# flkraus/bayesian-yolov3

Measured on AMD Instinct MI355X. Metric: img/s at T=30 MC-dropout, 608x608, higher is better.
Workload: dtype f32 via split-f16 (hi+lo fp16 pairs, 3 fp16 MFMA products, fp32 accumulate)

## Files before the change

### bayesian-yolov3_amd/byolo/_lib.py

```python
import ctypes
import os

_HERE = os.path.dirname(os.path.abspath(__file__))
LIB_PATH = os.environ.get("BYOLO_LIB") or os.path.join(_HERE, "libbyolo.so")

OK, ERR_ARG, ERR_STATE, ERR_HIP, ERR_NOMEM, ERR_RANGE = 0, -1, -2, -3, -4, -5
DET_STANDARD, DET_ALEATORIC, DET_EPISTEMIC = 0, 1, 2
NMS_AGNOSTIC, NMS_TWO_CLASS, NMS_PER_CLASS = 0, 1, 2
NMS_MAX_CLASSES = 128
NORM_BN, NORM_DROPOUT = 1, 2
AUG_SATURATION, AUG_BRIGHTNESS, AUG_HUE = 1, 2, 3
AUG_COLORED_SALT_N_PEPPER, AUG_SALT_N_PEPPER, AUG_GAUSSIAN = 1, 2, 3


class ByoloError(RuntimeError):
    def __init__(self, code, msg):
        super().__init__("libbyolo error %d: %s" % (code, msg))
        self.code = code


class Cfg(ctypes.Structure):
    _fields_ = [("img_h", ctypes.c_int32), ("img_w", ctypes.c_int32), ("img_c", ctypes.c_int32),
                ("cls_cnt", ctypes.c_int32), ("drop_prob", ctypes.c_float), ("max_out", ctypes.c_int32),
                ("iou_thresh", ctypes.c_float), ("nms_mode", ctypes.c_int32), ("keep_all_outputs", ctypes.c_int32)]


class PlanOpts(ctypes.Structure):
    _fields_ = [(n, ctypes.c_int32) for n in (
        "struct_bytes", "graphs", "serialize_convs", "serialize_heads", "dedup", "lowmain", "kx3", "p1", "b2b", "kx3_wide", "wino_split", "wino_split_min_c",
        "wino_split_bn", "wino_split_rounds", "winograd", "wino_fused", "stream1x1", "gemm_stream", "ksplit", "streamk",
        "plain_epilogue", "wshift_per_layer", "nms_general", "wino_split_persist", "wino_split_feed")] + [(n, ctypes.c_float) for n in (
        "wino_split_min_gflop", "wino_split_chunk_mb", "wino_min_gflop", "wino_chunk_mb", "wino_min_ratio")]


class AugPlan(ctypes.Structure):
    _fields_ = [(n, ctypes.c_int32) for n in ("y0", "x0", "ch", "cw", "row0", "rescale", "flip", "blur_k", "color_op", "noise_op")] + \
               [("color_param", ctypes.c_float), ("noise_param", ctypes.c_float), ("noise_key", ctypes.c_uint64)]


EVAL_MAX_GT, EVAL_MAX_UNC, EVAL_RECORD_HEAD = 1024, 16, 7


class EvalCfg(ctypes.Structure):
    _fields_ = [(n, ctypes.c_int32) for n in ("struct_bytes", "row_len", "obj_idx", "cls_start_idx", "cls_cnt", "n_unc")] + \
               [("unc_cols", ctypes.c_int32 * EVAL_MAX_UNC), ("iou_thresh", ctypes.c_float), ("min_score", ctypes.c_float)]


EVAL_LOC_WORDS, EVAL_LOC_MAX_LAYERS, EVAL_LOC_MAX_PRIORS = 6, 8, 16


class EvalLocCfg(ctypes.Structure):
    _fields_ = [(n, ctypes.c_int32) for n in ("struct_bytes", "layer_col", "prior_col", "n_layers")] + \
               [(n, ctypes.c_int32 * EVAL_LOC_MAX_LAYERS) for n in ("lh", "lw", "n_priors")] + \
               [(n, (ctypes.c_float * EVAL_LOC_MAX_PRIORS) * EVAL_LOC_MAX_LAYERS) for n in ("prior_w", "prior_h")]


EVAL_LADDER_MAX = 16


class EvalLadderCfg(ctypes.Structure):
    _fields_ = [("struct_bytes", ctypes.c_int32), ("n_thr", ctypes.c_int32), ("thresholds", ctypes.c_float * EVAL_LADDER_MAX)]


EVAL_SUBSETS_MAX = 16


class EvalSubsetsCfg(ctypes.Structure):
    _fields_ = [("struct_bytes", ctypes.c_int32), ("n_subsets", ctypes.c_int32), ("lo", ctypes.c_float * EVAL_SUBSETS_MAX),
                ("hi", ctypes.c_float * EVAL_SUBSETS_MAX), ("img_h", ctypes.c_float), ("ignore_thresh", ctypes.c_float),
                ("height_slack", ctypes.c_float), ("ignore_other_classes", ctypes.c_int32)]


class EvalSummary(ctypes.Structure):
    _fields_ = [(n, ctypes.c_int32) for n in ("struct_bytes", "overflow", "record_words", "reserved")] + \
               [(n, ctypes.c_int64) for n in ("n_records", "n_seen", "n_images")]


VOTE_NONE, VOTE_ALE, VOTE_EPI, VOTE_TOTAL = 0, 1, 2, 3


class VoteCfg(ctypes.Structure):
    _fields_ = [("struct_bytes", ctypes.c_int32), ("var", ctypes.c_int32)] + \
               [(n, ctypes.c_float) for n in ("sigma_t", "iou_min", "min_score", "var_floor")] + \
               [("ale_col", ctypes.c_int32), ("epi_col", ctypes.c_int32)]


SOFT_NMS_LINEAR, SOFT_NMS_GAUSSIAN = 0, 1
SOFT_NMS_RESIDENT = 8192


class SoftNmsCfg(ctypes.Structure):
    _fields_ = [("struct_bytes", ctypes.c_int32), ("method", ctypes.c_int32)] + \
               [(n, ctypes.c_float) for n in ("sigma", "iou_soft", "iou_hard", "min_score")]


VAR_RECAL_ALE, VAR_RECAL_EPI, VAR_RECAL_TOTAL = 1, 2, 3
VAR_RECAL_SCALE, VAR_RECAL_POWER = 0, 1
VAR_RECAL_FITTED, VAR_RECAL_SCALE_FALLBACK, VAR_RECAL_IDENTITY, VAR_RECAL_EMPTY = 0, 1, 2, 3
VAR_RECAL_TABLE_BYTES, VAR_RECAL_FIT_WORDS = 8192, 10


class VarRecalCfg(ctypes.Structure):
    _fields_ = [(n, ctypes.c_int32) for n in ("struct_bytes", "kind", "target", "n_layers")] + \
               [("n_priors", ctypes.c_int32 * EVAL_LOC_MAX_LAYERS)] + \
               [(n, ((ctypes.c_double * 4) * EVAL_LOC_MAX_PRIORS) * EVAL_LOC_MAX_LAYERS) for n in ("a", "b")]


SCORE_RECAL_MAX_K, SCORE_RECAL_MAX_GROUPS, SCORE_RECAL_TABLE_BYTES, SCORE_RECAL_FIT_WORDS = 8, 80, 5120, 36
SCORE_RECAL_BY_ALL, SCORE_RECAL_BY_CLASS = 0, 1
SCORE_RECAL_F_BIAS, SCORE_RECAL_F_LOGIT, SCORE_RECAL_F_LOG_HEIGHT, SCORE_RECAL_F_COL_ID, SCORE_RECAL_F_COL_LOG = 0, 1, 2, 3, 4
SCORE_RECAL_FIT, SCORE_RECAL_IDENTITY, SCORE_RECAL_EMPTY = 0, 1, 2


class ScoreRecalCfg(ctypes.Structure):
    _fields_ = [(n, ctypes.c_int32) for n in ("struct_bytes", "kind", "cls_cnt", "by", "K")] + \
               [(n, ctypes.c_int32 * SCORE_RECAL_MAX_K) for n in ("feat_kind", "feat_col")] + [("reserved", ctypes.c_int32)] + \
               [("w", (ctypes.c_double * SCORE_RECAL_MAX_K) * SCORE_RECAL_MAX_GROUPS)]


_i32, _i64, _f32 = ctypes.c_int32, ctypes.c_int64, ctypes.c_float
_vp, _cp, _sz, _u64 = ctypes.c_void_p, ctypes.c_char_p, ctypes.c_size_t, ctypes.c_uint64
_P = ctypes.POINTER

PROTOTYPES = {
    "byolo_create": (_i32, [_P(Cfg), _i32, _P(_vp)]),
    "byolo_destroy": (_i32, [_vp]),
    "byolo_last_error": (_cp, [_vp]),
    "byolo_version": (_cp, []),
    "byolo_add_conv": (_i32, [_vp, _cp, _i32, _i32, _i32, _i32]),
    "byolo_add_residual": (_i32, [_vp, _i32]),
    "byolo_add_route": (_i32, [_vp, _P(_i32), _i32]),
    "byolo_add_upsample": (_i32, [_vp]),
    "byolo_add_stack": (_i32, [_vp, _i32]),
    "byolo_add_detection": (_i32, [_vp, _cp, _i32, _P(_f32)]),
    "byolo_mark_backbone_end": (_i32, [_vp]),
    "byolo_num_params": (_i32, [_vp]),
    "byolo_param_info": (_i32, [_vp, _i32, _P(_cp), _P(_i32), _P(_i64)]),
    "byolo_set_param": (_i32, [_vp, _cp, _vp, _i64]),
    "byolo_get_param": (_i32, [_vp, _cp, _vp, _i64]),
    "byolo_finalize": (_i32, [_vp]),
    "byolo_num_layers": (_i32, [_vp]),
    "byolo_num_boxes": (_i32, [_vp, _P(_i64), _P(_i32)]),
    "byolo_workspace_bytes": (_i32, [_vp, _i32, _i32, _P(_sz)]),
    "byolo_forward": (_i32, [_vp, _vp, _i32, _i32, _u64, _i32, _vp, _vp, _sz, _vp, _vp, _vp, _vp, _vp]),
    "byolo_num_dropout": (_i32, [_vp]),
    "byolo_mask_layout": (_i32, [_vp, _i32, _i32, _i32, _P(_i64), _P(_i64)]),
    "byolo_set_async": (_i32, [_vp, _i32]),
    "byolo_status": (_i32, [_vp, _vp, _P(ctypes.c_uint32), _P(_i32)]),
    "byolo_clear_status": (_i32, [_vp, _vp]),
    "byolo_precision_note": (_cp, [_vp]),
    "byolo_set_first_image": (_i32, [_vp, _i64]),
    "byolo_max_images": (_i32, [_vp, _i32, _P(_i32)]),
    "byolo_layer_output": (_i32, [_vp, _i32, _P(_vp), _P(_i64)]),
    "byolo_copy_layer_output": (_i32, [_vp, _i32, _vp, _i64, _vp]),
    "byolo_set_precision": (_i32, [_vp, _i32]),
    "byolo_get_precision": (_i32, [_vp]),
    "byolo_decode": (_i32, [_vp, _i32, _vp, _i32, _i32, _i32, _i32, _P(_f32), _i32, _vp, _i64, _i64, _vp]),
    "byolo_epistemic_stats": (_i32, [_vp, _vp, _i32, _i32, _i32, _i32, _vp, _vp, _vp, _vp, _vp]),
    "byolo_nms_workspace_bytes": (_sz, [_i32, _i64]),
    "byolo_nms_workspace_bytes_ex": (_sz, [_i32, _i64, _i32, _i32]),
    "byolo_nms_class_counts": (_i32, [_vp, _vp, _i32, _i32, _vp]),
    "byolo_sort_nms": (_i32, [_vp, _vp, _i32, _i64, _i32, _i32, _i32, _i32, _i32, _f32, _vp, _sz, _vp, _vp, _vp, _vp]),
    "byolo_calibrate_bn": (_i32, [_vp, _vp, _i32, _vp, _sz, _vp]),
    "byolo_set_profiling": (_i32, [_vp, _i32]),
    "byolo_resume_profiling": (_i32, [_vp, _i32]),
    "byolo_stage_ms": (_i32, [_vp, _P(_f32)]),
    "byolo_set_profile_depth": (_i32, [_vp, _i32]),
    "byolo_select_profile": (_i32, [_vp, _i32]),
    "byolo_num_steps": (_i32, [_vp]),
    "byolo_step_profile": (_i32, [_vp, _i32, _P(_i32), _P(_i32), _P(_i64), _P(_f32), _P(ctypes.c_double)]),
    "byolo_step_split": (_i32, [_vp, _i32, _P(_i32), _P(_i32)]),
    "byolo_flops": (_i32, [_vp, _i32, _i32, _P(ctypes.c_double)]),
    "byolo_crc32c": (ctypes.c_uint32, [_vp, _sz]),
    "byolo_abi_version": (_i32, []),
    "byolo_get_plan_opts": (_i32, [_vp, _P(PlanOpts)]),
    "byolo_set_plan_opts": (_i32, [_vp, _P(PlanOpts)]),
    "byolo_graph_stats": (_i32, [_vp, _P(_i32), _P(_i64), _P(_i64), _P(_i64)]),
    "byolo_plan_num": (_i32, [_vp, _i32, _i32, _i32, _P(_i32), _P(_i32), _P(_i64)]),
    "byolo_plan_step": (_i32, [_vp, _i32, _P(_i32), _P(_i32), _P(_i32), _P(_i32)]),
    "byolo_plan_tensor": (_i32, [_vp, _i32, _P(_i64), _P(_i64), _P(_i32)]),
    "byolo_set_tshard": (_i32, [_vp, _i32, _i32]),
    "byolo_finish_tshard": (_i32, [_vp, _vp, _i32, _i32, _vp]),
    "byolo_normalize_u8": (_i32, [_vp, _vp, _i64, _vp, _vp]),
    "byolo_copy_status": (_i32, [_vp, _vp, _vp]),
# ... 92 lines not shown
```

### bayesian-yolov3_amd/csrc/byolo_api.hip

```cpp
#include "byolo_internal.h"
#include <cfloat>

static thread_local std::string g_err;

int32_t byolo_fail(byolo_t* h, int32_t code, const char* fmt, ...) {
    char buf[1024];
    va_list ap; va_start(ap, fmt); vsnprintf(buf, sizeof buf, fmt, ap); va_end(ap);
    if (h) h->err = buf; else g_err = buf;
    return code;
}

extern "C" const char* byolo_version(void) { return "byolo 0.7 (gfx950; fp32 MFMA and split-f16 MFMA; abi 7)"; }
extern "C" int32_t byolo_abi_version(void) { return BYOLO_ABI_VERSION; }

extern "C" const char* byolo_last_error(const byolo_t* h) { return h ? h->err.c_str() : g_err.c_str(); }

static void plan_opts_defaults(byolo_plan_opts& o);
static void plan_opts_from_env(byolo_plan_opts& o);

extern "C" int32_t byolo_create(const byolo_cfg* cfg, int32_t device, byolo_t** out) {
    if (!cfg || !out) return fail(nullptr, BYOLO_ERR_ARG, "byolo_create: null argument");
    if (cfg->img_h <= 0 || cfg->img_w <= 0 || cfg->img_c <= 0)
        return fail(nullptr, BYOLO_ERR_ARG, "byolo_create: invalid image size");
    if (cfg->img_h % 32 || cfg->img_w % 32)
        return fail(nullptr, BYOLO_ERR_ARG, "byolo_create: full_img_size must be a multiple of 32 (yolov3.py:207-208)");
    if (cfg->cls_cnt < 1 || cfg->cls_cnt > byk::BYOLO_MAX_CLASSES)
        return fail(nullptr, BYOLO_ERR_ARG, "byolo_create: cls_cnt outside 1 .. 128");
    if (cfg->max_out < 1 || cfg->max_out > 2048) return fail(nullptr, BYOLO_ERR_ARG, "byolo_create: max_out out of [1,2048]");
    if (!(cfg->drop_prob >= 0.f && cfg->drop_prob < 1.f)) return fail(nullptr, BYOLO_ERR_ARG, "byolo_create: drop_prob");
    byolo_t* h = new (std::nothrow) byolo();
    if (!h) return fail(nullptr, BYOLO_ERR_NOMEM, "byolo_create: out of host memory");
    h->cfg = *cfg;
    h->device = device;
    plan_opts_defaults(h->opts);
    plan_opts_from_env(h->opts);
    h->dedup = h->opts.dedup != 0;
    if (const char* e = getenv("BYOLO_PRECISION")) h->precision = (!strcmp(e, "f32") || !strcmp(e, "0")) ? 0 : 1;
    h->prec_requested = h->precision;
    *out = h;
    return BYOLO_OK;
}

static void plan_opts_defaults(byolo_plan_opts& o) {
    memset(&o, 0, sizeof o);
    o.struct_bytes = (int32_t)sizeof o;
    o.graphs = 1; o.serialize_convs = 1; o.serialize_heads = 1; o.dedup = 1; o.lowmain = 1; o.kx3 = 1; o.p1 = 1; o.b2b = 1; o.kx3_wide = 0;
    o.wino_split = 1; o.wino_split_min_c = 256; o.wino_split_bn = 0; o.wino_split_rounds = 0;
    o.winograd = 1; o.wino_fused = 1; o.stream1x1 = 1; o.gemm_stream = 1; o.ksplit = -1; o.streamk = 1; o.plain_epilogue = 1; o.wino_split_persist = 0; o.wino_split_feed = 3;
    o.wino_split_min_gflop = 30.f; o.wino_split_chunk_mb = 1500.f; o.wino_min_gflop = 10.f; o.wino_chunk_mb = 800.f; o.wino_min_ratio = 80.f;
}
static void plan_opts_from_env(byolo_plan_opts& o) {
    auto geti = [](const char* name, int32_t& v) { if (const char* e = getenv(name)) v = atoi(e); };
    auto getf = [](const char* name, float& v) { if (const char* e = getenv(name)) v = (float)atof(e); };
    geti("BYOLO_GRAPHS", o.graphs); geti("BYOLO_SERIALIZE_CONVS", o.serialize_convs); geti("BYOLO_SERIALIZE_HEADS", o.serialize_heads);
    if (const char* e = getenv("BYOLO_NO_DEDUP")) o.dedup = atoi(e) ? 0 : 1;
    geti("BYOLO_LOWMAIN", o.lowmain); geti("BYOLO_KX3", o.kx3); geti("BYOLO_P1", o.p1); geti("BYOLO_B2B", o.b2b); geti("BYOLO_KX3_WIDE", o.kx3_wide);
    geti("BYOLO_WINO_SPLIT", o.wino_split); geti("BYOLO_WINO_SPLIT_MIN_C", o.wino_split_min_c); geti("BYOLO_WINO_SPLIT_BN", o.wino_split_bn);
    geti("BYOLO_WINO_SPLIT_ROUNDS", o.wino_split_rounds); geti("BYOLO_WINOGRAD", o.winograd);
    geti("BYOLO_WINO_FUSED", o.wino_fused); geti("BYOLO_STREAM1X1", o.stream1x1); geti("BYOLO_GEMM_STREAM", o.gemm_stream);
    geti("BYOLO_KSPLIT", o.ksplit); geti("BYOLO_STREAMK", o.streamk); geti("BYOLO_PLAIN_EPILOGUE", o.plain_epilogue); geti("BYOLO_WINO_SPLIT_PERSIST", o.wino_split_persist); geti("BYOLO_WINO_SPLIT_FEED", o.wino_split_feed);
    geti("BYOLO_WSHIFT_PER_LAYER", o.wshift_per_layer); geti("BYOLO_NMS_GENERAL", o.nms_general);
    getf("BYOLO_WINO_SPLIT_MIN_GFLOP", o.wino_split_min_gflop); getf("BYOLO_WINO_SPLIT_CHUNK_MB", o.wino_split_chunk_mb);
    getf("BYOLO_WINO_MIN_GFLOP", o.wino_min_gflop); getf("BYOLO_WINO_CHUNK_MB", o.wino_chunk_mb); getf("BYOLO_WINO_MIN_RATIO", o.wino_min_ratio);
}

static void drop_graphs(byolo_t* h) {
    bool any = false;
    for (auto& g : h->graphs) any = any || g.exec;
    if (any) (void)hipDeviceSynchronize();
    for (auto& g : h->graphs) if (g.exec) (void)hipGraphExecDestroy(g.exec);
    h->graphs.clear();
}

extern "C" int32_t byolo_get_plan_opts(const byolo_t* h, byolo_plan_opts* out) {
    if (!h || !out) return fail(const_cast<byolo_t*>(h), BYOLO_ERR_ARG, "byolo_get_plan_opts: null argument");
    *out = h->opts;
    out->struct_bytes = (int32_t)sizeof *out;
    return BYOLO_OK;
}

extern "C" int32_t byolo_set_plan_opts(byolo_t* h, const byolo_plan_opts* o) {
    if (!h || !o) return fail(h, BYOLO_ERR_ARG, "byolo_set_plan_opts: null argument");
    if (o->struct_bytes != (int32_t)sizeof *o) return fail(h, BYOLO_ERR_ARG, "byolo_set_plan_opts: struct_bytes %d, this library's byolo_plan_opts has %d (include/byolo.h)", o->struct_bytes, (int)sizeof *o);
    if (o->graphs < 0 || o->graphs > 2 || o->serialize_convs < 0 || o->serialize_convs > 2 || o->b2b < 0 || o->b2b > 2 || o->kx3_wide < 0 || o->kx3_wide > 2 ||
        o->wino_split < 0 || o->wino_split > 2 || o->winograd < 0 || o->winograd > 2 || o->wino_fused < 0 || o->wino_fused > 2 || o->stream1x1 < 0 || o->stream1x1 > 2 ||
        o->streamk < 0 || o->streamk > 2 || o->ksplit < -1 || o->ksplit > 64 || (o->wino_split_bn != 0 && o->wino_split_bn != 128 && o->wino_split_bn != 256) ||
        o->wino_split_rounds < 0 || o->wino_split_persist < 0 || o->wino_split_persist > 2 || o->wino_split_feed < 0 || o->wino_split_feed > 3 || !(o->wino_split_chunk_mb > 0.f) || !(o->wino_chunk_mb > 0.f) || !(o->wino_split_min_gflop >= 0.f) || !(o->wino_min_gflop >= 0.f) || !(o->wino_min_ratio >= 0.f))
        return fail(h, BYOLO_ERR_ARG, "byolo_set_plan_opts: a field outside its range (include/byolo.h)");
    const byolo_plan_opts& c = h->opts;
    const bool repack = (o->wshift_per_layer != 0) != (c.wshift_per_layer != 0) || (o->dedup != 0) != (c.dedup != 0) || (o->lowmain != 0) != (c.lowmain != 0) || (o->kx3 != 0) != (c.kx3 != 0) || (o->p1 != 0) != (c.p1 != 0);
    h->opts = *o;
    h->dedup = o->dedup != 0;
    invalidate_plan(h);
    if (h->d_blob || !h->graphs.empty()) { HIPCHK(h, hipSetDevice(h->device)); drop_graphs(h); }
    if (repack && h->lowered) { h->lowered = false; h->finalized = false; }
    return BYOLO_OK;
}

extern "C" int32_t byolo_graph_stats(const byolo_t* h, int32_t* n_graphs, int64_t* replays, int64_t* captures, int64_t* updates) {
    if (!h) return BYOLO_ERR_ARG;
    int n = 0; for (const auto& g : h->graphs) n += g.exec != nullptr;
    if (n_graphs) *n_graphs = n;
    if (replays) *replays = h->graph_replays;
    if (captures) *captures = h->graph_captures;
    if (updates) *updates = h->graph_updates;
    return BYOLO_OK;
}

extern "C" int32_t byolo_set_precision(byolo_t* h, int32_t precision) {
    if (!h) return fail(nullptr, BYOLO_ERR_ARG, "byolo_set_precision: null handle");
    if (precision != BYOLO_PREC_F32 && precision != BYOLO_PREC_SPLIT_F16) return fail(h, BYOLO_ERR_ARG, "byolo_set_precision: unknown precision %d", precision);
    h->prec_requested = precision;
    if (precision == BYOLO_PREC_F32) h->prec_note.clear();
    if (precision != h->precision) { h->precision = precision; h->prec_note.clear(); h->finalized = false; h->plan.B = -1; h->plan.T = -1; ++h->plan_epoch; }
    return BYOLO_OK;
}
extern "C" int32_t byolo_get_precision(const byolo_t* h) { return h ? h->precision : BYOLO_ERR_ARG; }

extern "C" int32_t byolo_destroy(byolo_t* h) {
    if (!h) return BYOLO_OK;
    bool on_device = h->d_blob || h->d_ones || h->d_status || !h->graphs.empty() || h->cap_stream;
    for (auto& ps : h->prof) on_device = on_device || ps.ev[0] || !ps.step_ev.empty();
    if (on_device) {
        (void)hipSetDevice(h->device);
        drop_graphs(h);
        if (h->cap_stream) (void)hipStreamDestroy(h->cap_stream);
        if (h->d_blob) (void)hipFree(h->d_blob);
        if (h->d_ones) (void)hipFree(h->d_ones);
        if (h->d_zeros) (void)hipFree(h->d_zeros);
        if (h->ev_convs) (void)hipEventDestroy(h->ev_convs);
        if (h->d_status) (void)hipFree(h->d_status);
        if (h->pc_own) (void)hipFree(h->pc_own);
        if (h->vn_own) (void)hipFree(h->vn_own);
        if (h->vr.dev) (void)hipFree(h->vr.dev);
        if (h->sr.dev) (void)hipFree(h->sr.dev);
        if (h->sr_own) (void)hipFree(h->sr_own);
        if (h->h_status) (void)hipHostFree(h->h_status);
        for (auto& ps : h->prof) {
            for (auto& e : ps.ev) if (e) (void)hipEventDestroy(e);
            for (auto& e : ps.step_ev) (void)hipEventDestroy(e);
        }
    }
    delete h;
    return BYOLO_OK;
}

static int add_param(byolo_t* h, const std::string& name, std::vector<int64_t> shape, float fill) {
    if (h->pindex.count(name)) return -1;
    Param p; p.name = name; p.shape = std::move(shape);
    p.data.assign((size_t)p.count(), fill);
    h->params.push_back(std::move(p));
    h->pindex[name] = (int)h->params.size() - 1;
    return (int)h->params.size() - 1;
}

static int resolve_ref(const byolo_t* h, int r) {
    const int n = (int)h->layers.size();
    const int a = r < 0 ? n + r : r;
    return (a < 0 || a >= n) ? -2 : a;
}

static void input_shape(const byolo_t* h, int prev, int& C, int& H, int& W, bool& stacked) {
    if (prev < 0) { C = h->cfg.img_c; H = h->cfg.img_h; W = h->cfg.img_w; stacked = false; }
    else { const Layer& l = h->layers[prev]; C = l.C; H = l.H; W = l.W; stacked = l.stacked; }
}

static int32_t begin_add(byolo_t* h, const char* what) {
    if (!h) return fail(nullptr, BYOLO_ERR_ARG, "%s: null handle", what);
    if (h->lowered) return fail(h, BYOLO_ERR_STATE, "%s: graph is frozen after byolo_finalize", what);
    return BYOLO_OK;
}

static constexpr int MAX_CHANNELS = 1 << 16;
static constexpr int64_t MAX_KERNEL_WEIGHTS = (int64_t)1 << 28;

static int32_t add_conv_impl(byolo_t* h, const char* scope, int32_t filters, int32_t ksize, int32_t stride, int32_t norm_flags) {
    int32_t rc = begin_add(h, "byolo_add_conv"); if (rc) return rc;
    if (!scope || !(ksize == 1 || ksize == 3)) return fail(h, BYOLO_ERR_ARG, "byolo_add_conv: invalid kernel size");
    if (!(stride == 1 || stride == 2)) return fail(h, BYOLO_ERR_ARG, "byolo_add_conv: invalid strides");
    if (stride == 2 && ksize != 3) return fail(h, BYOLO_ERR_ARG, "byolo_add_conv: invalid kernel size (layers.py:629)");
    if (filters < 1) return fail(h, BYOLO_ERR_ARG, "byolo_add_conv: filters < 1");
    if (filters > MAX_CHANNELS) return fail(h, BYOLO_ERR_ARG, "byolo_add_conv: more than %d filters", MAX_CHANNELS);
    if (!(norm_flags & BYOLO_NORM_BN)) return fail(h, BYOLO_ERR_ARG, "byolo_add_conv: BN-less conv layers are not on this path");
    Layer l; l.op = OP_CONV; l.scope = scope; l.filters = filters; l.ksize = ksize; l.stride = stride; l.norm = norm_flags;
    l.prev = (int)h->layers.size() - 1;
    int C, H, W; bool st; input_shape(h, l.prev, C, H, W, st);
    if (stride == 2 && ((H | W) & 1)) return fail(h, BYOLO_ERR_ARG, "byolo_add_conv: stride 2 needs even input size");
    if ((int64_t)ksize * ksize * C * filters > MAX_KERNEL_WEIGHTS)
        return fail(h, BYOLO_ERR_ARG, "byolo_add_conv: a kernel of %lld weights (limit 2^28)", (long long)ksize * ksize * C * filters);
    l.Cin = C; l.C = filters; l.H = H / stride; l.W = W / stride; l.stacked = st;
    const std::string s(scope);
    l.p_kernel = add_param(h, s + "/conv2d/kernel", {ksize, ksize, C, filters}, 0.f);
    l.p_gamma = add_param(h, s + "/batch_normalization/gamma", {filters}, 1.f);
    l.p_beta = add_param(h, s + "/batch_normalization/beta", {filters}, 0.f);
    l.p_mean = add_param(h, s + "/batch_normalization/moving_mean", {filters}, 0.f);
    l.p_var = add_param(h, s + "/batch_normalization/moving_variance", {filters}, 1.f);
    if (l.p_kernel < 0 || l.p_gamma < 0) return fail(h, BYOLO_ERR_ARG, "byolo_add_conv: duplicate scope '%s'", scope);
    if (norm_flags & BYOLO_NORM_DROPOUT) l.drop_ordinal = h->n_dropout++;
    h->layers.push_back(l);
    return (int32_t)h->layers.size() - 1;
}
extern "C" int32_t byolo_add_conv(byolo_t* h, const char* scope, int32_t filters, int32_t ksize, int32_t stride,
                                  int32_t norm_flags) {
    return guarded(h, "byolo_add_conv", [&] { return add_conv_impl(h, scope, filters, ksize, stride, norm_flags); });
}

extern "C" int32_t byolo_add_residual(byolo_t* h, int32_t shortcut) {
    int32_t rc = begin_add(h, "byolo_add_residual"); if (rc) return rc;
    Layer l; l.op = OP_RESIDUAL; l.prev = (int)h->layers.size() - 1;
    const int a = resolve_ref(h, shortcut);
    if (a < 0 || l.prev < 0) return fail(h, BYOLO_ERR_ARG, "byolo_add_residual: bad shortcut %d", shortcut);
    const Layer& x = h->layers[l.prev]; const Layer& s = h->layers[a];
    if (x.C != s.C || x.H != s.H || x.W != s.W || x.stacked != s.stacked)
        return fail(h, BYOLO_ERR_ARG, "byolo_add_residual: shape mismatch");
    l.ref[0] = a; l.nref = 1; l.C = x.C; l.H = x.H; l.W = x.W; l.stacked = x.stacked;
    h->layers.push_back(l);
    return (int32_t)h->layers.size() - 1;
}

extern "C" int32_t byolo_add_route(byolo_t* h, const int32_t* routes, int32_t n) {
    int32_t rc = begin_add(h, "byolo_add_route"); if (rc) return rc;
    if (!routes || n >= 3) return fail(h, BYOLO_ERR_ARG, "byolo_add_route: too many routes");
    if (n < 1) return fail(h, BYOLO_ERR_ARG, "byolo_add_route: too few routes");
    Layer l; l.op = OP_ROUTE; l.prev = (int)h->layers.size() - 1; l.nref = n;
    for (int i = 0; i < n; ++i) {
        l.ref[i] = resolve_ref(h, routes[i]);
        if (l.ref[i] < 0) return fail(h, BYOLO_ERR_ARG, "byolo_add_route: bad route %d", routes[i]);
    }
    const Layer& a = h->layers[l.ref[0]];
    l.C = a.C; l.H = a.H; l.W = a.W; l.stacked = a.stacked;
    if (n == 2) {
        const Layer& b = h->layers[l.ref[1]];
        if (a.H != b.H || a.W != b.W || a.stacked != b.stacked)
            return fail(h, BYOLO_ERR_ARG, "byolo_add_route: concat shape mismatch");
        l.C = a.C + b.C;
        if (l.C > MAX_CHANNELS) return fail(h, BYOLO_ERR_ARG, "byolo_add_route: more than %d channels", MAX_CHANNELS);
    }
    h->layers.push_back(l);
    return (int32_t)h->layers.size() - 1;
}
// ... 319 lines not shown
    p.N = layer_pitch(l); p.Npad = st.Npad; p.ldc = layer_pitch(l);
    p.cin_tiles = (st.c_hi - st.c_lo) / 32; p.KT = l.ksize * l.ksize * p.cin_tiles;
    p.wpk = dptr(h, st.w_off);
    p.epi = raw_epi(h, st.layer);
    p.dst = h->plan.off[st.out_tensor] >= 0 ? reinterpret_cast<float*>(ws + h->plan.off[st.out_tensor]) : nullptr;
    p.src0_bytes = (uint32_t)((uint64_t)nsrc[0] * Hs[0] * Wsz[0] * Cs[0] * 4);
    p.src1_bytes = Cs[1] ? (uint32_t)((uint64_t)nsrc[1] * Hs[1] * Wsz[1] * Cs[1] * 4) : p.src0_bytes;
    p.w_bytes = (uint32_t)((uint64_t)p.KT * p.Npad * 32 * 4);
    p.d_hw = make_fastdiv((uint32_t)(p.Hout * p.Wout)); p.d_wout = make_fastdiv((uint32_t)p.Wout);
    p.d_sdiv0 = make_fastdiv((uint32_t)sdiv[0]); p.d_sdiv1 = make_fastdiv((uint32_t)sdiv[1]);
    p.rep = st.mode == STEP_REP ? T : 1;
    p.split = h->precision != 1 ? 0 : (!l.direct ? 1 : ((l.prev >= 0 ? 1 : 0) | (l.op == OP_DETECTION ? 0 : 2)));
    if (p.split && st.kx3) { p.kx3 = 1; p.KT = 3 * p.cin_tiles; }
    else if (p.split && st.p1) p.kx3 = 2;
    if (st.mode == STEP_MAIN) {
        p.addend = reinterpret_cast<const float*>(ws + h->plan.off[st.addend_tensor]);
        p.addend_T = l.stacked ? T : 1;
    } else { p.addend = nullptr; p.addend_T = 1; }
    p.d_addT = make_fastdiv((uint32_t)p.addend_T);
    p.no_plain = h->opts.plain_epilogue == 0;
}

static void fill_finish(const byolo_t* h, const Step& st, char* ws, int B, int T, int mode, FinishParams& f) {
    const Layer& l = h->layers[st.layer];
    memset(&f, 0, sizeof f);
    f.low = reinterpret_cast<const float*>(ws + h->plan.off[st.low_tensor]);
    f.part = st.addend_tensor >= 0 ? reinterpret_cast<const float*>(ws + h->plan.off[st.addend_tensor]) : nullptr;
    f.dst = h->plan.off[st.out_tensor] >= 0 ? reinterpret_cast<float*>(ws + h->plan.off[st.out_tensor]) : nullptr;
    f.T = l.stacked ? T : 1; f.S = B * f.T; f.H = l.H; f.W = l.W; f.N = l.filters;
    f.mode = mode;
    f.epi = raw_epi(h, st.layer); f.epi.flags = 0;
    f.d_hw = make_fastdiv((uint32_t)(l.H * l.W / 4)); f.d_w = make_fastdiv((uint32_t)(l.W / 2));
    f.d_n4 = make_fastdiv((uint32_t)(l.filters / 4)); f.d_T = make_fastdiv((uint32_t)f.T);
}

static int32_t run_aux_step(byolo_t* h, const Step& s, const ConvParams& p, hipStream_t st) {
    const Layer& l = h->layers[s.layer];
    if (s.mode == STEP_GATHER) { HIPCHK(h, launch_view_gather(p, st)); }
    else { HIPCHK(h, launch_tensor_add(p.src0, p.src1, p.dst, (int64_t)p.M * l.C, h->precision == 1, st, p.epi.status, s.layer)); }
    return BYOLO_OK;
}

static int32_t next_event(byolo_t* h, hipStream_t st, int* idx) {
    byolo::ProfSlot& ps = h->wslot();
    while ((int)ps.step_ev.size() <= ps.n_ev) { hipEvent_t e; HIPCHK(h, hipEventCreate(&e)); ps.step_ev.push_back(e); }
    HIPCHK(h, hipEventRecord(ps.step_ev[ps.n_ev], st));
    *idx = ps.n_ev++;
    return BYOLO_OK;
}

static int32_t mark_launch(byolo_t* h, int layer, int variant, int64_t m, int64_t n, int64_t k, double algo, hipStream_t st,
                           int ksplit = 1, int split_tiles = 0) {
    byolo::ProfSlot& ps = h->wslot();
    int e; int32_t rc = next_event(h, st, &e); if (rc) return rc;
    if (ps.last_main >= 0) ps.launches[ps.last_main].ev_end = e;
    ps.last_main = (int)ps.launches.size();
    ps.launches.push_back({layer, variant, m, n, k, algo, ksplit, split_tiles, e, -1});
    return BYOLO_OK;
}

static int32_t run_winograd(byolo_t* h, const Step& s, const Layer& l, const ConvParams& c, const WinoPlan& wp, int tile,
                            double algo_flops, char* ws, hipStream_t st) {
    const bool prof = h->profiling >= 2;
    int32_t rc;
    const int S = c.M / (l.H * l.W), tt = wp.th * wp.tw;
    float* V = reinterpret_cast<float*>(ws + h->plan.wino_off);
    float* Mb = reinterpret_cast<float*>(ws + h->plan.wino_off + wp.v_bytes);
    for (int s0 = 0; s0 < S; s0 += wp.chunk) {
        const int ns = std::min(wp.chunk, S - s0);
        WinoParams w; memset(&w, 0, sizeof w);
        w.x = c.src0; w.v = V; w.m = Mb; w.y = c.dst;
        w.residual = (c.epi.flags & EPI_RESIDUAL) ? c.residual : nullptr;
        w.epi = c.epi;
        w.H = l.H; w.W = l.W; w.C = c.C0; w.N = c.N; w.th = wp.th; w.tw = wp.tw;
        w.s0 = s0; w.P = ns * tt; w.P_pad = (int)align_up((size_t)w.P, 128);
        w.d_tt = make_fastdiv((uint32_t)tt); w.d_tw = make_fastdiv((uint32_t)wp.tw);
        w.d_c4 = make_fastdiv((uint32_t)(c.C0 / 4)); w.d_n4 = make_fastdiv((uint32_t)(c.N / 4));
        if (prof && (rc = mark_launch(h, s.layer, -2, w.P, c.C0, 0, 0.0, st))) return rc;
        HIPCHK(h, launch_wino_input(w, st));

        const int rows = 16 * w.P_pad;
        if (wp.fused) {
            WinoFusedParams f; memset(&f, 0, sizeof f);
            f.v = V; f.v_bytes = (uint32_t)((uint64_t)rows * c.C0 * 4);
            f.w = dptr(h, s.wino_off); f.wstride = (uint32_t)((size_t)(c.C0 / 32) * c.N * 32 * 4); f.w_bytes = 16u * f.wstride;
            f.y = c.dst; f.residual = w.residual; f.epi = c.epi;
            f.C = c.C0; f.N = c.N; f.KT = c.C0 / 32; f.n_tiles = c.N / 64;
            f.H = l.H; f.W = l.W; f.th = wp.th; f.tw = wp.tw; f.s0 = s0; f.P = w.P;
            const int RT = w.P_pad / 128;
            f.slots = 512 / f.n_tiles; f.q = RT / f.slots; f.rem = RT % f.slots;
            f.xi_stride = (uint32_t)((uint64_t)w.P_pad * c.C0 * 4);
            f.d_ntiles = make_fastdiv((uint32_t)f.n_tiles); f.d_tt = w.d_tt; f.d_tw = w.d_tw;
            if (prof && (rc = mark_launch(h, s.layer, 130, rows, c.N, c.C0, algo_flops * ns / S, st))) return rc;
            HIPCHK(h, launch_wino_fused(f, st));
            continue;
        }
        if (h->opts.gemm_stream != 0 && gemm_stream_ok(c.C0, c.N)) {
            GemmStreamParams q; memset(&q, 0, sizeof q);
            q.a = V; q.a_bytes = (uint32_t)((uint64_t)rows * c.C0 * 4);
            q.w = dptr(h, s.wino_off); q.wstride = (uint32_t)((size_t)(c.C0 / 32) * c.N * 32 * 4); q.w_bytes = 16u * q.wstride;
            q.dst = Mb; q.C = c.C0; q.N = c.N; q.KT = c.C0 / 32; q.n_tiles = c.N / 128;
            q.RT = w.P_pad / 128;
            const int R = 16 * q.RT;
            q.slots = 512 / q.n_tiles; q.q = R / q.slots; q.rem = R % q.slots;
            q.d_ntiles = make_fastdiv((uint32_t)q.n_tiles); q.d_RT = make_fastdiv((uint32_t)q.RT);
            q.kind = 0; q.epi = raw_epi(h, s.layer); q.M = rows; q.Npad = c.N; q.ldc = c.N;
            if (prof && (rc = mark_launch(h, s.layer, 129, rows, c.N, c.C0, algo_flops * ns / S, st))) return rc;
            HIPCHK(h, launch_gemm_stream(q, st));
            if (prof && (rc = mark_launch(h, s.layer, -3, w.P, c.N, 0, 0.0, st))) return rc;
            HIPCHK(h, launch_wino_output(w, st));
            continue;
        }
        ConvParams g; memset(&g, 0, sizeof g);
        g.src0 = V; g.src1 = V; g.C0 = c.C0; g.C1 = 0;
        g.src0_bytes = g.src1_bytes = (uint32_t)((uint64_t)rows * c.C0 * 4);
        g.Hs0 = g.Hs1 = 1; g.Ws0 = g.Ws1 = rows; g.sdiv0 = g.sdiv1 = 1;
        g.Hin = 1; g.Win = rows; g.Hout = 1; g.Wout = rows; g.ksize = 1; g.stride = 1; g.pad = 0;
        g.M = rows; g.N = c.N; g.Npad = c.Npad; g.ldc = c.N; g.cin_tiles = c.C0 / 32; g.KT = g.cin_tiles;
        g.wpk = dptr(h, s.wino_off);
        g.wino_rows = (uint32_t)w.P_pad; g.d_wino = make_fastdiv((uint32_t)w.P_pad);
        g.wino_wstride = (uint32_t)((size_t)g.cin_tiles * c.Npad * 32 * 4);
        g.w_bytes = 16u * g.wino_wstride;
        g.epi = raw_epi(h, s.layer); g.rep = 1; g.addend_T = 1;
        g.dst = Mb;
        g.d_hw = make_fastdiv((uint32_t)rows); g.d_wout = make_fastdiv((uint32_t)rows);
        g.d_sdiv0 = g.d_sdiv1 = g.d_addT = make_fastdiv(1u);
        const ConvSplit sp = conv_plan_split(rows, c.Npad, g.KT, tile, 1.0, h->opts.ksplit, h->opts.streamk);
        if (conv_split_slab_bytes(sp, tile) <= h->plan.slab_bytes) {
            g.full_tiles = sp.full_tiles; g.split_tiles = sp.split_tiles; g.split_blocks = sp.split_blocks; g.ksplit = sp.ksplit;
            g.sk_grid = sp.sk_grid;
            g.slabs = c.slabs; g.slab_bytes = (uint32_t)conv_split_slab_bytes(sp, tile); g.counters = c.counters;
        }
        if (prof && (rc = mark_launch(h, s.layer, conv_tile_bn(tile), rows, c.N, c.C0, algo_flops * ns / S, st, g.sk_grid > 0 ? -g.sk_grid : (g.ksplit > 1 ? g.ksplit : 1), g.split_tiles))) return rc;
        HIPCHK(h, launch_conv_igemm(g, tile, st));
        if (prof && (rc = mark_launch(h, s.layer, -3, w.P, c.N, 0, 0.0, st))) return rc;
        HIPCHK(h, launch_wino_output(w, st));
    }
    return BYOLO_OK;
}

static int32_t run_wino_split(byolo_t* h, const Step& s, const Layer& l, const ConvParams& c, const WinoPlan& wp, double algo_flops,
                              char* ws, hipStream_t st, const WinoParams* feed = nullptr) {
    const bool prof = h->profiling >= 2;
    int32_t rc;
    const int S = c.M / (l.H * l.W), tt = wp.th * wp.tw;
    float* V = reinterpret_cast<float*>(ws + h->plan.wino_off);
    const bool drop = c.epi.flags & EPI_DROPOUT;
    for (int s0 = 0; s0 < S; s0 += wp.chunk) {
        const int ns = std::min(wp.chunk, S - s0);
        WinoParams w; memset(&w, 0, sizeof w);
        if (feed) w = *feed;
        w.x = feed ? nullptr : c.src0; w.v = V;
        w.H = l.H; w.W = l.W; w.C = c.C0; w.N = c.N; w.th = wp.th; w.tw = wp.tw;
        w.s0 = s0; w.P = ns * tt; w.P_pad = (int)align_up((size_t)w.P, 128);
        w.d_tt = make_fastdiv((uint32_t)tt); w.d_tw = make_fastdiv((uint32_t)wp.tw);
        w.d_c4 = make_fastdiv((uint32_t)(c.C0 / 4)); w.d_n4 = make_fastdiv((uint32_t)(c.N / 4));
        w.vmul = 1.f / ACT_SCALE;
        if (prof && (rc = mark_launch(h, s.layer, -4, w.P, c.C0, 0, 0.0, st))) return rc;
        HIPCHK(h, launch_wino_split_input(w, st));
        WinoSplitParams f; memset(&f, 0, sizeof f);
        const uint64_t rows = (uint64_t)16 * w.P_pad;
        f.v = V; f.v_bytes = (uint32_t)(rows * c.C0 * 4); f.xi_stride = (uint32_t)((uint64_t)w.P_pad * c.C0 * 4);
        f.w = dptr(h, s.wino_off); f.w_bytes = (uint32_t)((size_t)16 * c.C0 * c.N * 4);
        f.y = c.dst; f.residual = (c.epi.flags & EPI_RESIDUAL) ? c.residual : nullptr;
        f.epi = c.epi; f.epi.scale = dptr(h, drop ? l.wscalek_off : l.wscale_off);
        f.C = c.C0; f.N = c.N; f.KT = c.C0 / 32; f.n_tiles = c.N / wp.bn; f.bn = wp.bn;
        f.H = l.H; f.W = l.W; f.th = wp.th; f.tw = wp.tw; f.s0 = s0; f.P = w.P; f.P_pad = w.P_pad;
        f.bm = wp.bm; f.units = (w.P_pad / wp.bm) * f.n_tiles;
        const int chunk_idx = s0 / wp.chunk;
        f.persist = (h->opts.wino_split_persist == 2 && c.counters && chunk_idx < CNT_PER_STEP / 8) ? 2 : (h->opts.wino_split_persist ? 1 : 0);
        f.claims = c.counters ? c.counters + 8 * chunk_idx : nullptr;
        f.d_ntiles = make_fastdiv((uint32_t)f.n_tiles); f.d_tt = w.d_tt; f.d_tw = w.d_tw;
        if (prof && (rc = mark_launch(h, s.layer, 140, (int64_t)rows, c.N, c.C0, algo_flops * ns / S, st, 1, wp.bn))) return rc;
        HIPCHK(h, launch_wino_split(f, st));
    }
    return BYOLO_OK;
}

static int32_t run_decode(byolo_t* h, char* ws, float* boxes, int B, int T, hipStream_t st, int mode = 0) {
    for (const auto& l : h->layers) {
        if (l.op != OP_DETECTION) continue;
        DecodeParams d; memset(&d, 0, sizeof d);
        d.mode = mode;
        if (mode && l.det_kind != BYOLO_DET_EPISTEMIC) return fail(h, BYOLO_ERR_ARG, "T sharding (byolo_set_tshard) is defined for epistemic detection layers");
        d.raw = mode == 2 ? nullptr : reinterpret_cast<const float*>(ws + h->plan.off[l.out_tensor]);
        d.boxes = boxes; d.lh = l.H; d.lw = l.W; d.C = h->cfg.cls_cnt;
        d.n_total = h->n_boxes; d.box_base = l.box_base; d.layer_id = l.det_id; d.ld = layer_pitch(l);
        d.status = h->precision == 1 ? h->d_status : nullptr;
        for (int k = 0; k < 3; ++k) { d.ph[k] = l.priors[2 * k]; d.pw[k] = l.priors[2 * k + 1]; }
        if (l.det_kind == BYOLO_DET_EPISTEMIC) { d.B = B; d.T = l.stacked ? T : 1; }
        else { d.B = l.stacked ? B * T : B; d.T = 1; }
        if (l.det_kind != BYOLO_DET_EPISTEMIC && l.stacked && T > 1)
            return fail(h, BYOLO_ERR_ARG, "byolo_forward: non-epistemic decode of a stacked (T>1) detection layer");
        HIPCHK(h, launch_decode(l.det_kind, d, st));
    }
    return BYOLO_OK;
}

static int64_t mask_layout(const byolo_t* h, int B, int T, int ordinal, int64_t* elements) {
    int64_t off = 0;
    for (const auto& l : h->layers) {
        if (l.drop_ordinal < 0) continue;
        const int64_t n = (l.stacked ? (int64_t)B * T : B) * l.H * l.W * l.filters;
        if (l.drop_ordinal == ordinal) { if (elements) *elements = n; return off; }
        off += (n + 31) / 32 * 32;
    }
    if (elements) *elements = 0;
    return off;
}

extern "C" int32_t byolo_num_dropout(const byolo_t* h) { return h ? h->n_dropout : BYOLO_ERR_ARG; }

static int32_t mask_layout_impl(byolo_t* h, int32_t B, int32_t T, int32_t ordinal, int64_t* bit_offset, int64_t* elements) {
    if (!h) return fail(nullptr, BYOLO_ERR_ARG, "byolo_mask_layout: null handle");
    if (!h->lowered) { int32_t rc = lower(h); if (rc) return rc; }
    if (B < 1 || T < 1 || ordinal < 0 || ordinal > h->n_dropout) return fail(h, BYOLO_ERR_ARG, "byolo_mask_layout: bad argument");
    int64_t n = 0;
    const int64_t off = mask_layout(h, B, T, ordinal, &n);
    if (bit_offset) *bit_offset = off;
    if (elements) *elements = n;
    return BYOLO_OK;
}
extern "C" int32_t byolo_mask_layout(byolo_t* h, int32_t B, int32_t T, int32_t ordinal, int64_t* bit_offset, int64_t* elements) {
    return guarded(h, "byolo_mask_layout", [&] { return mask_layout_impl(h, B, T, ordinal, bit_offset, elements); });
}

static int32_t read_status(byolo_t* h, hipStream_t st, unsigned* flags, unsigned* layer) {
    if (!h->d_status) { *flags = 0; *layer = 0xFFFFFFFFu; return BYOLO_OK; }
    HIPCHK(h, hipMemcpyAsync(h->h_status, h->d_status, 2 * sizeof(unsigned), hipMemcpyDeviceToHost, st));
    HIPCHK(h, hipStreamSynchronize(st));
    *flags = h->h_status[0]; *layer = h->h_status[1];
    return BYOLO_OK;
}
static int32_t range_error(byolo_t* h, const char* what, unsigned flags, unsigned layer) {
    const char* scope = layer < h->layers.size() ? h->layers[layer].scope.c_str() : "?";
    if (flags & 1u)
        return fail(h, BYOLO_ERR_RANGE, "%s: an output of layer %u ('%s') exceeds the split-f16 range (|activation| > %.0f); the reference's float32 "
                    "tensor (lib_yolo/layers.py:550) holds it -- run this model with byolo_set_precision(BYOLO_PREC_F32)", what, layer, scope, 65504.0 / ACT_SCALE);
    return fail(h, BYOLO_ERR_RANGE, "%s: a raw detection output is inf / NaN (non-finite activations upstream, or weights the float32 reference overflows on as well)", what);
}

extern "C" int32_t byolo_set_async(byolo_t* h, int32_t on) {
    if (!h) return fail(nullptr, BYOLO_ERR_ARG, "byolo_set_async: null handle");
    h->async_status = on != 0;
    return BYOLO_OK;
}

extern "C" int32_t byolo_status(byolo_t* h, void* stream, uint32_t* flags, int32_t* layer) {
    if (!h) return fail(nullptr, BYOLO_ERR_ARG, "byolo_status: null handle");
    if (!h->finalized) return fail(h, BYOLO_ERR_STATE, "byolo_status: call byolo_finalize first");
    HIPCHK(h, hipSetDevice(h->device));
    unsigned f = 0, l = 0xFFFFFFFFu;
    int32_t rc = read_status(h, reinterpret_cast<hipStream_t>(stream), &f, &l); if (rc) return rc;
    if (flags) *flags = f;
    if (layer) *layer = (f & 1u) ? (int32_t)l : -1;
    return f ? range_error(h, "byolo_status", f, l) : BYOLO_OK;
}

extern "C" int32_t byolo_clear_status(byolo_t* h, void* stream) {
    if (!h) return fail(nullptr, BYOLO_ERR_ARG, "byolo_clear_status: null handle");
    if (!h->d_status) return BYOLO_OK;
    HIPCHK(h, hipSetDevice(h->device));
    hipStream_t st = reinterpret_cast<hipStream_t>(stream);
    HIPCHK(h, hipMemsetAsync(h->d_status, 0, sizeof(unsigned), st));
    HIPCHK(h, hipMemsetAsync(h->d_status + 1, 0xFF, sizeof(unsigned), st));
    return BYOLO_OK;
}

extern "C" int32_t byolo_copy_status(byolo_t* h, uint32_t* d_out, void* stream) {
    if (!h || !d_out) return fail(h, BYOLO_ERR_ARG, "byolo_copy_status: null argument");
    if (!h->finalized) return fail(h, BYOLO_ERR_STATE, "byolo_copy_status: call byolo_finalize first");
    HIPCHK(h, hipSetDevice(h->device));
    hipStream_t st = reinterpret_cast<hipStream_t>(stream);
    if (!h->d_status) { HIPCHK(h, hipMemsetAsync(d_out, 0, 2 * sizeof(uint32_t), st)); return BYOLO_OK; }
    HIPCHK(h, hipMemcpyAsync(d_out, h->d_status, 2 * sizeof(uint32_t), hipMemcpyDeviceToDevice, st));
    return BYOLO_OK;
}

extern "C" int32_t byolo_normalize_u8(byolo_t* h, const uint8_t* d_u8, int64_t n, float* d_f32, void* stream) {
    if (!h || n < 0 || (n > 0 && (!d_u8 || !d_f32))) return fail(h, BYOLO_ERR_ARG, "byolo_normalize_u8: bad argument");
    if ((reinterpret_cast<uintptr_t>(d_u8) & 3) || (reinterpret_cast<uintptr_t>(d_f32) & 15))
        return fail(h, BYOLO_ERR_ARG, "byolo_normalize_u8: d_u8 must be 4-byte and d_f32 16-byte aligned");
    if (n == 0) return BYOLO_OK;
    HIPCHK(h, hipSetDevice(h->device));
    HIPCHK(h, launch_u8_to_f32(d_u8, d_f32, n, reinterpret_cast<hipStream_t>(stream)));
    return BYOLO_OK;
}

extern "C" const char* byolo_precision_note(const byolo_t* h) { return h ? h->prec_note.c_str() : ""; }

static int32_t forward_piece(byolo_t* h, const float* d_img, int32_t B, int32_t T, uint64_t seed, int32_t dropout_on,
                             const uint32_t* d_mask_bits, void* d_workspace, size_t workspace_bytes, float* d_boxes, float* d_rows,
                             int32_t* d_kept, int32_t* d_count, void* stream);
static SoftNmsParams soft_params(const byolo_soft_nms_cfg& c);
struct FwdArgs { const float* d_img; int32_t B, T; uint64_t seed; int32_t dropout_on; const uint32_t* d_mask_bits; void* d_workspace;
                 float* d_boxes; float* d_rows; int32_t* d_kept; int32_t* d_count; };
static int32_t enqueue_forward(byolo_t* h, const FwdArgs& a, hipStream_t st, bool capturing, bool wait_convs, bool heads_only = false);
static int32_t finish_forward(byolo_t* h, hipStream_t st, void* stream);
static int32_t forward_graph(byolo_t* h, const FwdArgs& a, hipStream_t st, bool* done);

static int32_t forward_impl(byolo_t* h, const float* d_img, int32_t B, int32_t T, uint64_t seed, int32_t dropout_on,
                                 const uint32_t* d_mask_bits, void* d_workspace, size_t workspace_bytes, float* d_boxes, float* d_rows,
                                 int32_t* d_kept, int32_t* d_count, void* stream) {
    if (h && h->finalized && B >= 1 && T >= 1) {
        if (!h->lowered) { int32_t rc = lower(h); if (rc) return rc; }
        const int64_t cap = piece_cap(h, T);
        if (cap >= 1 && B > cap) {
            if (d_mask_bits && dropout_on)
                return fail(h, BYOLO_ERR_ARG, "byolo_forward: injected masks describe ONE piece: keep B <= byolo_max_images (%lld at T = %d)", (long long)cap, T);
            const int64_t first = h->first_image;
            const size_t img_el = (size_t)h->cfg.img_h * h->cfg.img_w * h->cfg.img_c;
            const bool per_class = h->cfg.nms_mode == BYOLO_NMS_PER_CLASS && d_rows;
            const size_t out_cap = (size_t)h->cfg.max_out * (h->cfg.nms_mode == BYOLO_NMS_TWO_CLASS ? 2 : h->cfg.nms_mode == BYOLO_NMS_PER_CLASS ? h->cfg.cls_cnt : 1);
            const size_t cc = (size_t)h->cfg.cls_cnt;
            if (per_class && h->pc_own_cap < (size_t)B * cc) {
                HIPCHK(h, hipSetDevice(h->device));
                if (h->pc_own) { HIPCHK(h, hipDeviceSynchronize()); HIPCHK(h, hipFree(h->pc_own)); h->pc_own = nullptr; h->pc_own_cap = 0; }
                HIPCHK(h, hipMalloc(reinterpret_cast<void**>(&h->pc_own), (size_t)B * cc * sizeof(int32_t)));
                h->pc_own_cap = (size_t)B * cc;
            }
// ... 881 lines not shown
```

### bayesian-yolov3_amd/csrc/byolo_kernels.h

```cpp
#pragma once
#include <hip/hip_runtime.h>
#include <stdint.h>
#include <atomic>

namespace byk {

inline hipError_t set_dynamic_lds_once(const void* fn, size_t bytes, std::atomic<uint64_t>& done) {
    int dev = 0;
    hipError_t e = hipGetDevice(&dev);
    if (e != hipSuccess) return e;
    const uint64_t bit = 1ull << (dev & 63);
    if (done.load(std::memory_order_acquire) & bit) return hipSuccess;
    e = hipFuncSetAttribute(fn, hipFuncAttributeMaxDynamicSharedMemorySize, (int)bytes);
    if (e == hipSuccess) done.fetch_or(bit, std::memory_order_release);
    return e;
}


enum : int { EPI_LEAKY = 1, EPI_DROPOUT = 2, EPI_RESIDUAL = 4, EPI_RAW = 8 ,
              EPI_F32OUT = 16  };
struct EpiArgs {
    const float* scale; const float* shift;
    const uint32_t* mask_bits;
    unsigned* status;
    uint64_t idx_base;
    uint32_t k0, k1, thr;
    int flags;
    int layer_idx;
};

struct FastDiv { uint32_t mul, shr; };
inline FastDiv make_fastdiv(uint32_t d) {
    uint32_t l = 0;
    while (l < 32 && ((uint64_t)1 << l) < d) ++l;
    FastDiv f;
    f.mul = (uint32_t)(((((uint64_t)1 << l) - d) << 32) / d + 1);
    f.shr = l;
    return f;
}

static constexpr uint32_t CONV_OOB_OFFSET = 0xC0000000u;
static constexpr uint64_t CONV_MAX_SRC_BYTES = 0xBFF00000ull;

struct ConvParams {
    const float* src0; const float* src1;
    uint32_t src0_bytes, src1_bytes;
    const float* wpk;
    uint32_t w_bytes;
    EpiArgs epi;
    const float* residual;
    const float* addend;
    int addend_T;
    int rep;
    float* dst;
    int C0, C1;
    int Hs0, Ws0, Hs1, Ws1;
    int sh0, sh1;
    int sdiv0, sdiv1;
    int Hin, Win, Hout, Wout;
    int ksize, stride, pad;
    int M, N, Npad, ldc;
    int KT, cin_tiles;
    int split;
    int kx3;
    int plain;
    int no_plain;
    FastDiv d_hw, d_wout, d_sdiv0, d_sdiv1, d_addT;
    int full_tiles, split_tiles, split_blocks, ksplit;
    int sk_grid, sk_q, sk_r;
    FastDiv d_skq, d_skq1, d_kt;
    float* slabs;
    uint32_t slab_bytes;
    unsigned* counters;
    uint32_t wino_rows, wino_wstride;
    FastDiv d_wino;
    FastDiv d_ntiles, d_cin, d_ks, d_ksplit;
    const float* f_wpk; uint32_t f_w_bytes;
    EpiArgs f_epi;
    float* f_dst;
    int f_N, f_Npad, f_ldc;
};

struct WinoParams {
    const float* x; float* v;
    const float* m; float* y;
    const float* residual;
    EpiArgs epi;
    int H, W, C, N, th, tw;
    int s0;
    int P, P_pad;
    FastDiv d_tt, d_tw, d_c4, d_n4;
    float vmul;
    int feed, src_T;
    const float* src_low; const float* src_part;
    EpiArgs src;
};
struct WinoSplitParams {
    const float* v; uint32_t v_bytes;
    uint32_t xi_stride;
    const float* w; uint32_t w_bytes;
    float* y;
    const float* residual;
    EpiArgs epi;
    int C, N, KT, n_tiles;
    int H, W, th, tw, s0, P, P_pad;
    int bm, bn;
    int persist;
    unsigned* claims;
    int units;
    FastDiv d_ntiles, d_tt, d_tw;
};
bool wino_split_ok(int C, int N);
hipError_t launch_wino_split_input(const WinoParams& p, hipStream_t st);
hipError_t launch_wino_split(const WinoSplitParams& p, hipStream_t st);
struct GemmStreamParams {
    const float* a; uint32_t a_bytes;
    const float* w; uint32_t w_bytes;
    float* dst;
    int C, N, KT, n_tiles;
    int RT;
    int slots, q, rem;
    uint32_t wstride;
    FastDiv d_ntiles, d_RT;
    int kind, M, Npad, ldc;
    EpiArgs epi;
    const float* addend; int hw;
    FastDiv d_hw, d_addT;
};
int conv1x1_stream_tile(int M, int C, int N, bool force = false);
struct WinoFusedParams {
    const float* v; uint32_t v_bytes;
    const float* w; uint32_t w_bytes;
    float* y; const float* residual;
    EpiArgs epi;
    int C, N, KT, n_tiles;
    int H, W, th, tw, s0, P;
    int slots, q, rem;
    uint32_t xi_stride, wstride;
    FastDiv d_ntiles, d_tt, d_tw;
};
bool wino_fused_ok(int C, int N);
hipError_t launch_wino_fused(const WinoFusedParams& p, hipStream_t st);
bool gemm_stream_ok(int C, int N);
hipError_t launch_gemm_stream(const GemmStreamParams& p, hipStream_t st);
hipError_t launch_wino_input(const WinoParams& p, hipStream_t st);
hipError_t launch_side_delay(int microseconds, hipStream_t st);
hipError_t launch_wino_output(const WinoParams& p, hipStream_t st);
void wino_weight_transform(const float g[9], float u[16]);

struct ConvSplit { int full_tiles, split_tiles, split_blocks, ksplit; int sk_grid = 0; };
ConvSplit conv_plan_split(int M, int Npad, int KT, int tile, double tk_scale = 1.0, int ksplit_knob = -1, int streamk_knob = 1);
size_t conv_split_slab_bytes(const ConvSplit& sp, int tile);

enum : int { TILE_128x128 = 0, TILE_128x64 = 1, TILE_128x32 = 2, TILE_128x256 = 3 };
int conv_tile_bn(int tile);
int conv_pick_tile(int N);
int conv_split_tile(int tile, bool wide);
hipError_t launch_conv_igemm(const ConvParams& p, int tile, hipStream_t st);
hipError_t launch_view_gather(const ConvParams& p, hipStream_t st);
hipError_t launch_tensor_add(const float* a, const float* b, float* dst, int64_t n, bool split, hipStream_t st, unsigned* status = nullptr, int layer = 0);
hipError_t launch_zero_words(void* p, int64_t n_words, hipStream_t st);
hipError_t launch_u8_to_f32(const uint8_t* src, float* dst, int64_t n, hipStream_t st);
hipError_t launch_f32_to_split(const float* src, float* dst, int64_t n, float mul, hipStream_t st, unsigned* status = nullptr);
hipError_t launch_split_to_f32(const float* src, float* dst, int64_t n, float mul, hipStream_t st);
hipError_t launch_conv_direct(const ConvParams& p, hipStream_t st);
struct FinishParams {
    const float* low; const float* part; float* dst;
    int S, H, W, N, T;
    EpiArgs epi;
    int mode;
    FastDiv d_hw, d_w, d_n4, d_T;
};
hipError_t launch_finish_upsampled(const FinishParams& p, hipStream_t st);

hipError_t launch_channel_stats(const float* x, int64_t M, int C, float* d_mean, float* d_var, double* d_tmp,
                                hipStream_t st);
hipError_t launch_bn_act_inplace(float* x, int64_t M, int C, const float* scale, const float* shift,
                                 const float* residual, int leaky, bool split, hipStream_t st, unsigned* status = nullptr, int layer = 0);
hipError_t launch_fold_bn(const float* gamma, const float* beta, const float* mean, const float* var, float eps,
                          float* scale, float* shift, int C, hipStream_t st);

constexpr int BYOLO_MAX_CLASSES = 128;
struct DecodeParams {
    const float* raw;
    float* boxes;
    int B, T, lh, lw, C;
    int64_t n_total, box_base;
    float ph[3], pw[3];
    int layer_id;
    int ld;
    unsigned* status;
    int mode;
};
hipError_t launch_decode(int kind, const DecodeParams& p, hipStream_t st);
hipError_t launch_epi_stats(const DecodeParams& p, float* ev_loc, float* covar, float* obj_s, float* cls_s, hipStream_t st);

size_t nms_workspace_bytes(int B, int64_t N, int C);
struct NmsParams {
    const float* boxes;
    int B; int64_t N; int D, obj_idx, cls_start;
    int C;
    int max_out; float iou_thr;
    void* ws; size_t ws_bytes;
    float* rows; int32_t* kept; int32_t* count;
    int general_only;
};
const int32_t* nms_class_counts_ptr(void* ws, int B, int64_t N, int C);
hipError_t launch_sort_nms(const NmsParams& p, hipStream_t st);

constexpr int SOFT_NMS_RESIDENT_CAP = 8192;
constexpr int SOFT_NMS_LINEAR = 0, SOFT_NMS_GAUSSIAN = 1;
struct SoftNmsParams {
    NmsParams n;
    int method;
    float sigma, iou_soft, iou_hard, min_score;
};
size_t soft_nms_workspace_bytes(int B, int64_t N, int C);
const int32_t* soft_nms_class_counts_ptr(void* ws, int B, int64_t N, int C);
hipError_t launch_soft_nms(const SoftNmsParams& p, hipStream_t st);

struct VoteGeom { int layer_col, prior_col, n_layers; int lh[8], lw[8], n_priors[8]; };
struct VoteParams {
    const float* boxes;
    int B; int64_t N; int D, obj_idx, cls_start;
    int C;
    int var;
    float sigma_t, iou_min, min_score, var_floor;
    int ale_col, epi_col;
    VoteGeom geom;
    const float* rows_in; const int32_t* kept; const int32_t* count; int cap;
    float* rows_out;
    int32_t* vote_n;
    void* ws; size_t ws_bytes;
};
size_t box_vote_workspace_bytes(int B, int64_t N);
hipError_t launch_box_vote(const VoteParams& p, hipStream_t st);

struct VarRecalParams {
    const float* in; float* out;
    int64_t n; int D;
    int kind, target;
    int n_layers, n_priors[8];
    const double* tab;
};
hipError_t launch_var_recal(const VarRecalParams& p, hipStream_t st);

struct ScoreRecalParams {
    const float* in; float* out;
    const int32_t* count;
    float* score;
    int B, cap, D;
    int obj_idx, cls_start, C;
    int by_class, K;
    int feat_kind[8], feat_col[8];
    const double* tab;
};
hipError_t launch_score_recal(const ScoreRecalParams& p, hipStream_t st);

struct EncodeGtParams {
    const float* boxes;
    const int32_t* labels;
    const int32_t* counts;
    int B, max_boxes, n_layers, N;
// ... 22 lines not shown
```

### bayesian-yolov3_amd/csrc/byolo_plan.hip

```cpp
#include "byolo_internal.h"

int layer_pitch(const Layer& l) { return (l.op == OP_DETECTION && !l.direct) ? (l.C + 3) / 4 * 4 : l.C; }

int64_t tensor_bytes(const byolo_t* h, int id, int B, int T) {
    const int n = (int)h->layers.size();
    if (id >= n) {
        const AuxTensor& a = h->aux[id - n];
        return (int64_t)align_up((size_t)((int64_t)B * (a.stacked ? T : 1) * a.H * a.W * a.C) * sizeof(float), 256);
    }
    const Layer& l = h->layers[id];
    const int64_t S = l.stacked ? (int64_t)B * T : B;
    return (int64_t)align_up((size_t)(S * l.H * l.W * layer_pitch(l)) * sizeof(float), 256);
}

void step_geometry(const byolo_t* h, const Step& st, int B, int T, int* M, int* KT) {
    const Layer& l = h->layers[st.layer];
    const bool per_image = st.mode == STEP_REP || (st.mode == STEP_PARTIAL && !st.low);
    const int64_t S = (l.stacked && !per_image) ? (int64_t)B * T : B;
    *M = (int)(S * (l.H >> (st.low ? 1 : 0)) * (l.W >> (st.low ? 1 : 0)));
    *KT = l.ksize * l.ksize * ((st.c_hi - st.c_lo) / 32);
}

void decide_loops(byolo_t* h) {
    const bool kx3_on = h->opts.kx3 != 0, p1_on = h->opts.p1 != 0;
    for (auto& st : h->steps) {
        st.kx3 = false; st.p1 = false;
        if (!st.is_conv()) continue;
        const Layer& l = h->layers[st.layer];
        if (l.direct || h->precision != 1) continue;
        st.kx3 = kx3_on && l.ksize == 3 && l.stride == 1 && st.in.n == 1 && st.in.s[0].sh == 0 && st.in.s[0].layer >= 0 && st.Npad >= 64 &&
                 (st.mode == STEP_NORMAL || st.mode == STEP_REP);
        st.p1 = p1_on && l.ksize == 1 && l.stride == 1 && st.in.n == 1 && st.in.s[0].layer >= 0 && st.Npad >= 64;
    }
}

void make_plan(byolo_t* h, int B, int T, bool inject) {
    Plan& p = h->plan;
    if (p.B == B && p.T == T && h->plan_inject == inject) return;
    h->plan_inject = inject;
    const int n = (int)h->layers.size() + (int)h->aux.size();
    p.B = B; p.T = T; p.off.assign(n, -1);
    struct Blk { int64_t off, size; };
    std::vector<Blk> free_list;
    int64_t end = 0;
    auto alloc = [&](int64_t sz) -> int64_t {
        for (size_t i = 0; i < free_list.size(); ++i) {
            if (free_list[i].size >= sz) {
                const int64_t o = free_list[i].off;
                free_list[i].off += sz; free_list[i].size -= sz;
                if (!free_list[i].size) free_list.erase(free_list.begin() + i);
                return o;
            }
        }
        if (!free_list.empty() && free_list.back().off + free_list.back().size == end) {
            const int64_t o = free_list.back().off; end = o + sz; free_list.pop_back(); return o;
        }
        const int64_t o = end; end += sz; return o;
    };
    auto release = [&](int64_t off, int64_t sz) {
        Blk b{off, sz};
        auto it = std::lower_bound(free_list.begin(), free_list.end(), b, [](const Blk& x, const Blk& y) { return x.off < y.off; });
        it = free_list.insert(it, b);
        if (it + 1 != free_list.end() && it->off + it->size == (it + 1)->off) { it->size += (it + 1)->size; free_list.erase(it + 1); }
        if (it != free_list.begin() && (it - 1)->off + (it - 1)->size == it->off) { (it - 1)->size += it->size; free_list.erase(it); }
    };
    p.fuse.assign(h->steps.size(), 0);
    { const int b2b = h->opts.b2b;
      for (size_t si = 0; b2b && h->precision == 1 && !inject && !h->cfg.keep_all_outputs && si + 1 < h->steps.size(); ++si) {
          const Step& s = h->steps[si];
          const Layer& l = h->layers[s.layer];
          if (!(s.is_conv() && s.kx3 && s.mode == STEP_NORMAL && l.op == OP_CONV && !l.direct && l.filters == 256 && s.Npad == 256 && l.fused_residual < 0)) continue;
          int M, KT; step_geometry(h, s, B, T, &M, &KT);
          if (b2b < 2 && (int64_t)((M + 127) / 128) < 4 * 256) continue;
          const Step& s2 = h->steps[si + 1];
          const Layer& l2 = h->layers[s2.layer];
          const int out_t = s.out_tensor;
          if (s2.is_conv() && s2.mode == STEP_NORMAL && s2.p1 && !l2.direct && l2.ksize == 1 && l2.stride == 1 && s2.in.n == 1 &&
              s2.in.s[0].layer == out_t && !s2.in.s[0].tile && s2.in.s[0].sh == 0 && s2.in.s[0].C == 256 && s2.c_lo == 0 && s2.c_hi == 256 &&
              l2.fused_residual < 0 && s2.Npad <= 128 && (layer_pitch(l2) % 4) == 0 && l2.H == l.H && l2.W == l.W && l2.stacked == l.stacked &&
              h->last_use[out_t] == (int)si + 1)
              p.fuse[si] = 1;
      }
    }
    p.wino.assign(h->steps.size(), WinoPlan{});
    size_t wino_scratch = 0;
    if (h->precision == 1) {
        const int on = h->opts.wino_split;
        const double min_flops = on >= 2 ? 0.0 : (double)h->opts.wino_split_min_gflop * 1e9, budget = (double)h->opts.wino_split_chunk_mb * 1e6;
        const int bm = 64;
        const int bn_pref = h->opts.wino_split_bn;
        auto model_ms = [](int64_t row_tiles, int N, int C, int bn) -> double {
            if (bn == 256) return (double)((row_tiles * (N / 256) + 255) / 256) * (0.030 + 0.000293 * C);
            const int64_t units = row_tiles * (N / 128), full = units / 512, rem = units % 512;
            const double t = (double)full * (0.012 + 0.000367 * C) + (rem == 0 ? 0.0 : rem <= 256 ? 0.024 + 0.00022 * C : 0.012 + 0.000367 * C);
            return units > 1024 ? 1.09 * t : t;
        };
        for (size_t si = 0; on && si < h->steps.size(); ++si) {
            const Step& s = h->steps[si];
            const Layer& l = h->layers[s.layer];
            if (!s.wino_ok || !s.kx3 || s.mode != STEP_NORMAL || !wino_split_ok(s.c_hi - s.c_lo, l.filters) || s.Npad != l.filters || (l.fused_residual >= 0 && l.drop_ordinal >= 0) || p.fuse[si]) continue;
            int M, KT; step_geometry(h, s, B, T, &M, &KT);
            const double flops = 2.0 * M * l.filters * 9.0 * l.Cin;
            if (flops < min_flops) continue;
            if (on < 2 && l.Cin < h->opts.wino_split_min_c) continue;
            const int th = (l.H + 1) / 2, tw = (l.W + 1) / 2, S = M / (l.H * l.W);
            const double per_sample = 16.0 * th * tw * l.Cin * 4.0;
            const int nchunks = std::max(1, (int)std::ceil(S * per_sample / budget));
            const int chunk = (S + nchunks - 1) / nchunks;
            const int64_t row_tiles = (int64_t)align_up((size_t)chunk * th * tw, 128) / bm;
            const bool can256 = (l.filters % 256) == 0;
            int bn = (bn_pref == 256 && can256) ? 256 : bn_pref == 128 ? 128 : 0;
            if (bn_pref == 256 && !can256) bn = 128;
            const double t256 = can256 ? model_ms(row_tiles, l.filters, l.Cin, 256) : 1e30, t128 = model_ms(row_tiles, l.filters, l.Cin, 128);
            if (bn == 0) bn = t256 <= t128 ? 256 : 128;
            if (on < 2) {
                const double t_res = l.fused_residual >= 0 ? 4.0 * M * l.filters / 2.5e9 : 0.0;
                const double t_wino = nchunks * ((bn == 256 ? t256 : t128) + 0.012 + (double)row_tiles * bm * per_sample / ((double)th * tw) / 4.5e9) + t_res;
                const double t_direct = 0.028 + flops / ((l.Cin >= 512 ? 390.0 : 425.0) * 1e9);
                if (t_wino > 0.97 * t_direct) continue;
            }
            WinoPlan& w = p.wino[si];
            w.th = th; w.tw = tw; w.bm = bm; w.fused = true;
            w.bn = bn;
            w.chunk = chunk;
            const int rounds = h->opts.wino_split_rounds;
            if (rounds > 0) {
                const int slots = (w.bn == 256 ? 256 : 512), n_tiles = l.filters / w.bn;
                const int64_t row_tiles = (int64_t)rounds * slots / n_tiles;
                const int tt = w.th * w.tw;
                int c = (int)((row_tiles * w.bm) / tt);
                while (c > 1 && (int64_t)align_up((size_t)c * tt, 128) / w.bm * n_tiles > (int64_t)rounds * slots) --c;
                w.chunk = std::max(1, std::min(S, c));
            }
            const size_t P_pad = align_up((size_t)w.chunk * w.th * w.tw, 128);
            w.v_bytes = align_up((size_t)16 * P_pad * l.Cin * 4, 256);
            if (w.v_bytes > CONV_MAX_SRC_BYTES) { w = WinoPlan{}; continue; }
            w.m_bytes = 0;
            wino_scratch = std::max(wino_scratch, w.v_bytes);
        }
    }
    p.feed.assign(h->steps.size(), 0); p.feed_src.assign(h->steps.size(), -1);
    std::vector<int> last_use = h->last_use;
    if (h->precision == 1 && h->opts.wino_split_feed && !h->cfg.keep_all_outputs) {
        std::vector<int> readers(n, 0);
        for (const Step& s : h->steps) {
            for (int k = 0; k < s.in.n; ++k) if (s.in.s[k].layer >= 0) ++readers[s.in.s[k].layer];
            if (s.addend_tensor >= 0) ++readers[s.addend_tensor];
            if (s.low_tensor >= 0) ++readers[s.low_tensor];
            const Layer& l = h->layers[s.layer];
            if (s.is_conv() && l.fused_residual >= 0) ++readers[h->layers[l.fused_residual].ref[0]];
        }
        for (int si = 0; si < (int)h->steps.size(); ++si) {
            const Step& s = h->steps[si];
            const int kind = s.mode == STEP_REP ? 1 : s.mode == STEP_FINISH ? 2 : 0;
            if (!kind || !(h->opts.wino_split_feed & kind) || (kind == 1 && s.raw_tensor < 0) || (kind == 2 && (s.low_tensor < 0 || s.addend_tensor < 0))) continue;
            const Layer& l = h->layers[s.layer];
            const int t = s.out_tensor, ri = h->last_use[t];
            if (t >= (int)h->layers.size() || l.op != OP_CONV || l.direct || l.fused_residual >= 0 || (l.filters & 3) || readers[t] != 1 || ri <= si) continue;
            const Step& r = h->steps[ri];
            if (p.wino[ri].chunk <= 0 || !r.wino_ok || r.in.n != 1 || r.in.s[0].layer != t || r.in.s[0].sh != 0 || r.in.s[0].tile) continue;
            p.feed[si] = (char)kind; p.feed_src[ri] = si;
            if (kind == 1) last_use[s.raw_tensor] = ri;
            else { last_use[s.low_tensor] = ri; if (s.addend_tensor >= 0) last_use[s.addend_tensor] = ri; }
        }
    }
    for (int si = 0; si < (int)h->steps.size(); ++si) {
        const Layer& l = h->layers[h->steps[si].layer];
        const int t = p.feed[si] == 1 ? h->steps[si].raw_tensor : h->steps[si].out_tensor;
        if (!(si > 0 && p.fuse[si - 1]) && p.feed[si] != 2) p.off[t] = alloc(tensor_bytes(h, t, B, T));
        if (p.fuse[si]) { const int t2 = h->steps[si + 1].out_tensor; p.off[t2] = alloc(tensor_bytes(h, t2, B, T)); }
        if (h->cfg.keep_all_outputs) continue;
        for (int k = 0; k < n; ++k)
            if (p.off[k] >= 0 && last_use[k] == si) release(p.off[k], tensor_bytes(h, k, B, T));
        if (last_use[t] < 0 && l.op != OP_DETECTION && p.feed[si] != 2) release(p.off[t], tensor_bytes(h, t, B, T));
    }
    p.arena = align_up((size_t)end, 256);
    p.boxes_off = p.arena;
    size_t o = p.boxes_off + align_up((size_t)B * h->n_boxes * h->row_len * sizeof(float), 256);
    p.nms_off = o; o += align_up(nms_workspace_bytes_ex(B, h->n_boxes, h->cfg.nms_mode, h->cfg.cls_cnt), 256);
    p.soft_off = o;
    if (h->soft_on) o += align_up(soft_nms_workspace_bytes(B, h->n_boxes, nms_classes(h->cfg.nms_mode, h->cfg.cls_cnt)), 256);
    p.vote_n_off = p.vote_off = o;
    if (h->vote_on) {
        o += align_up((size_t)B * nms_out_cap(h) * sizeof(int32_t), 256);
        p.vote_off = o; o += align_up(box_vote_workspace_bytes(B, h->n_boxes), 256);
    }
    p.score_off = o;
    if (h->sr.on) o += align_up((size_t)B * nms_out_cap(h) * sizeof(float), 256);
    p.stats_off = o; o += align_up((size_t)1024 * 2 * h->maxC * sizeof(double) + 2 * h->maxC * sizeof(float), 256);
    p.img_split_off = o; if (h->img_split) o += align_up((size_t)B * h->cfg.img_h * h->cfg.img_w * h->cfg.img_c * sizeof(float), 256);
    p.split.assign(h->steps.size(), ConvSplit{0, 0, 0, 1});
    p.tile.assign(h->steps.size(), 0);
    size_t slab = 0;
    for (size_t si = 0; si < h->steps.size(); ++si) {
        const Step& s = h->steps[si];
        const Layer& l = h->layers[s.layer];
        if (!s.is_conv() || l.direct) continue;
        int M, KT; step_geometry(h, s, B, T, &M, &KT);
        int tile = s.tile;
        if (tile == TILE_128x128 && (l.filters % 128) == 0 && (int64_t)((M + 127) / 128) * (l.filters / 128) < 512) tile = TILE_128x64;
        if (h->precision == 1) tile = conv_split_tile(tile, s.kx3 || s.p1);
        else if (inject && tile == TILE_128x128) tile = TILE_128x64;
        const int kx3_wide = h->opts.kx3_wide;
        if (h->precision == 1 && s.kx3 && (s.Npad % 256) == 0 && kx3_wide && (l.filters % 128) == 0 &&
            (kx3_wide >= 2 ? (tile == TILE_128x128 || tile == TILE_128x64)
                           : (tile == TILE_128x128 && (int64_t)((M + 127) / 128) * (s.Npad / 256) >= 4 * 256)))
            tile = TILE_128x256;
        if (p.fuse[si]) tile = TILE_128x256;
        p.tile[si] = tile;
        const bool sp = h->precision == 1, kx3 = sp && s.kx3;
        p.split[si] = conv_plan_split(M, s.Npad, kx3 ? KT / 3 : KT, tile, sp ? (kx3 ? 1.2 : 0.4) : 1.0, h->opts.ksplit, h->opts.streamk);
        if (s.low) p.split[si] = ConvSplit{((M + 127) / 128) * (s.Npad / conv_tile_bn(tile)), 0, 0, 1};
        if (tile == TILE_128x256) p.split[si] = ConvSplit{((M + 127) / 128) * (s.Npad / 256), 0, 0, 1};
        slab = std::max(slab, conv_split_slab_bytes(p.split[si], tile));
    }
    { const int on = (h->precision == 1 || inject) ? 0 : h->opts.winograd;
      const double min_flops = on >= 2 ? 0.0 : (double)h->opts.wino_min_gflop * 1e9, budget = (double)h->opts.wino_chunk_mb * 1e6;
      for (size_t si = 0; on && si < h->steps.size(); ++si) {
        const Step& s = h->steps[si];
        const Layer& l = h->layers[s.layer];
        if (!s.wino_ok) continue;
        int M, KT; step_geometry(h, s, B, T, &M, &KT);
        if (2.0 * M * l.filters * 9.0 * l.Cin < min_flops) continue;
        const double min_ratio = (double)h->opts.wino_min_ratio;
        if (on < 2 && (double)l.Cin * l.filters / (l.Cin + l.filters) < min_ratio) continue;
        WinoPlan& w = p.wino[si];
        w.th = (l.H + 1) / 2; w.tw = (l.W + 1) / 2;
        const int S = M / (l.H * l.W);
        const double per_sample = 16.0 * w.th * w.tw * (l.Cin + l.filters) * 4.0;
        const int nchunks = (int)std::ceil(S * per_sample / budget);
        w.chunk = (S + nchunks - 1) / nchunks;
        const int fused_mode = h->opts.wino_fused;
        if (fused_mode && wino_fused_ok(l.Cin, l.filters)) {
            const int slots = 512 / (l.filters / 64), tt = w.th * w.tw;
            const int max_c = (int)std::max(1.0, std::min((double)S, std::floor(budget / (16.0 * tt * l.Cin * 4.0))));
            auto rt = [&](int c) { return (c * tt + 127) / 128; };
            auto rounds = [&](int c) { return (rt(c) + slots - 1) / slots; };
            int best_c = 0; double best_cost = 1e30;
            for (int c = std::max(1, max_c / 6); c <= max_c; ++c) {
                const int full = S / c, last = S % c;
                const double cost = full * (rounds(c) + 0.15) + (last ? rounds(last) + 0.15 : 0.0);
                if (cost < best_cost - 1e-9 || (std::fabs(cost - best_cost) < 1e-9 && c > best_c)) { best_cost = cost; best_c = c; }
            }
            if (best_c > 0 && (fused_mode >= 2 || rt(best_c) / slots >= 3)) { w.fused = true; w.chunk = best_c; }
        }
        const size_t P_pad = align_up((size_t)w.chunk * w.th * w.tw, 128);
        w.v_bytes = align_up((size_t)16 * P_pad * l.Cin * 4, 256);
        w.m_bytes = w.fused ? 0 : align_up((size_t)16 * P_pad * l.filters * 4, 256);
        wino_scratch = std::max(wino_scratch, w.v_bytes + w.m_bytes);
        const int rows = (int)(16 * P_pad);
        p.split[si] = conv_plan_split(rows, s.Npad, l.Cin / 32, s.tile, 1.0, h->opts.ksplit, h->opts.streamk);
        p.tile[si] = s.tile;
        slab = std::max(slab, conv_split_slab_bytes(p.split[si], s.tile));
      }
    }
    p.stream1x1.assign(h->steps.size(), 0);
    { const bool on = h->precision == 0 && !inject && h->opts.stream1x1 != 0, force = h->opts.stream1x1 >= 2;
      for (size_t si = 0; on && si < h->steps.size(); ++si) {
        const Step& s = h->steps[si];
        const Layer& l = h->layers[s.layer];
        if (!s.is_conv() || l.direct || l.ksize != 1 || l.stride != 1) continue;
        if (s.mode != STEP_NORMAL && s.mode != STEP_MAIN) continue;
        if (s.in.n != 1 || s.in.s[0].sh || s.in.s[0].tile || s.in.s[0].layer < 0 || l.fused_residual >= 0) continue;
        if (l.op == OP_CONV && (l.filters % 4)) continue;
        int M, KT; step_geometry(h, s, B, T, &M, &KT);
        const int bn = conv1x1_stream_tile(M, s.c_hi - s.c_lo, l.filters, force);
        if (bn && (l.filters <= 64 ? s.Npad == 64 : s.Npad == l.filters)) p.stream1x1[si] = bn;
      }
    }
    p.wino_off = o; o += align_up(wino_scratch, 256);
    p.slab_off = o; p.slab_bytes = slab; o += align_up(slab, 256);
    p.cnt_bytes = h->steps.size() * CNT_PER_STEP * sizeof(unsigned);
    p.cnt_off = o; o += align_up(p.cnt_bytes, 256);
    p.total = o;
}

extern "C" int32_t byolo_num_layers(const byolo_t* h) { return h ? (int32_t)h->layers.size() : BYOLO_ERR_ARG; }

extern "C" int32_t byolo_num_boxes(const byolo_t* h, int64_t* n, int32_t* d) {
    if (!h) return BYOLO_ERR_ARG;
    if (n) *n = h->n_boxes;
    if (d) *d = h->row_len;
    return BYOLO_OK;
}

int64_t piece_cap(const byolo_t* h, int32_t T) {
    uint64_t per_image = (uint64_t)h->cfg.img_h * h->cfg.img_w * h->cfg.img_c * 4;
// ... 99 lines not shown
```

### bayesian-yolov3_amd/csrc/wino_split.hip

```cpp
#include <hip/hip_runtime.h>
#include <type_traits>
#include "byolo_kernels.h"
#include "byolo_rng.h"
#include "mfma_pipe.h"
#include "epilogue.h"

namespace byk {

using namespace pipe;

#ifndef BYOLO_WS_ABLATE
#define BYOLO_WS_ABLATE 0
#endif
static constexpr int WS_ABL = BYOLO_WS_ABLATE;
#ifndef BYOLO_WS_FOLD_SKIP
#define BYOLO_WS_FOLD_SKIP 1
#endif
static constexpr bool WS_FOLD_SKIP = BYOLO_WS_FOLD_SKIP != 0;
#ifndef BYOLO_WS_RES_AHEAD
#define BYOLO_WS_RES_AHEAD 1
#endif

#ifndef BYOLO_WS_V_KTMAJOR
#define BYOLO_WS_V_KTMAJOR 1
#endif
__device__ __forceinline__ size_t v_index(uint32_t t, uint32_t c, uint32_t C) {
    if constexpr (BYOLO_WS_V_KTMAJOR != 0) return ((size_t)((t >> 6) * (C >> 5) + (c >> 5)) * 64u + (t & 63u)) * 32u + (c & 31u);
    else return (size_t)t * C + c;
}
#ifndef BYOLO_WS_IN_COLMAJOR
#define BYOLO_WS_IN_COLMAJOR 1
#endif
#ifndef BYOLO_WS_NT_STORE
#define BYOLO_WS_NT_STORE 1
#endif
__device__ __forceinline__ void vstore(float* at, const f32x4 v) {
    if constexpr (BYOLO_WS_NT_STORE != 0) __builtin_nontemporal_store(v, reinterpret_cast<f32x4*>(at));
    else *reinterpret_cast<f32x4*>(at) = v;
}
#ifndef BYOLO_WS_FEED_SLICE
#define BYOLO_WS_FEED_SLICE 5
#endif
template <int FEED, int DROP>
__global__ __launch_bounds__(256) void wino_split_input2_kernel(const WinoParams p, const FastDiv d_twp, const FastDiv d_ttp, const int twp, const FastDiv d_th,
                                                                const uint32_t groups, const uint32_t img_lo, const FastDiv d_nsl, const uint32_t nsl) {
    const uint32_t gid = blockIdx.x * 256u + threadIdx.x;
    const uint32_t c4n = (uint32_t)p.C >> 2;
    const uint32_t q = fdiv(gid, p.d_c4), c4 = gid - q * c4n;
    const size_t xi_stride = (size_t)p.P_pad * p.C;
    const uint32_t ttp = (uint32_t)(p.th * twp), n_pairs = groups * ttp;
    if (q >= n_pairs) {
        const uint32_t t = (uint32_t)p.P + (q - n_pairs);
        if (t >= (uint32_t)p.P_pad) return;
        float* v = p.v + v_index(t, c4 * 4, (uint32_t)p.C);
#pragma unroll
        for (int k = 0; k < 16; ++k) vstore(v + (size_t)k * xi_stride, f32x4{0.f, 0.f, 0.f, 0.f});
        return;
    }
    const uint32_t s = fdiv(q, d_ttp), r = q - s * ttp;
    uint32_t ty, txp;
    if constexpr (BYOLO_WS_IN_COLMAJOR != 0) { txp = fdiv(r, d_th); ty = r - txp * (uint32_t)p.th; }
    else { ty = fdiv(r, d_twp); txp = r - ty * (uint32_t)twp; }
    constexpr uint32_t PAIR = FEED == 1 ? 1u : 2u;
    const uint32_t tx0 = PAIR * txp;
    const bool two = PAIR == 2u && tx0 + 1u < (uint32_t)p.tw;
    const int y0 = 2 * (int)ty - 1, x0 = 2 * (int)tx0 - 1;
    const float m = p.vmul;
    auto emit_tile = [&](const uint32_t sl, const f32x4 (&u)[4][6], const int k) __attribute__((always_inline)) {
        const uint32_t t0 = ((sl * (uint32_t)p.th + ty) * (uint32_t)p.tw + tx0);
        float* v = p.v + v_index(t0 + (uint32_t)k, c4 * 4, (uint32_t)p.C);
        const int o = 2 * k;
#pragma unroll
        for (int i = 0; i < 4; ++i) {
            vstore(v + (size_t)(i * 4 + 0) * xi_stride, epi::split_encode4((u[i][o + 0] - u[i][o + 2]) * m));
            vstore(v + (size_t)(i * 4 + 1) * xi_stride, epi::split_encode4((u[i][o + 1] + u[i][o + 2]) * m));
            vstore(v + (size_t)(i * 4 + 2) * xi_stride, epi::split_encode4((u[i][o + 2] - u[i][o + 1]) * m));
            vstore(v + (size_t)(i * 4 + 3) * xi_stride, epi::split_encode4((u[i][o + 1] - u[i][o + 3]) * m));
        }
    };
    auto emit = [&](const uint32_t sl, const f32x4 (&u)[4][6]) __attribute__((always_inline)) {
        emit_tile(sl, u, 0);
        if (two) emit_tile(sl, u, 1);
    };
    auto column = [&](f32x4 (&u)[4][6], const int j, const f32x4 (&d)[4]) __attribute__((always_inline)) {
        u[0][j] = d[0] - d[2];
        u[1][j] = d[1] + d[2];
        u[2][j] = d[2] - d[1];
        u[3][j] = d[1] - d[3];
    };
    if constexpr (FEED == 0) {
        const float* img = p.x + ((size_t)(p.s0 + s) * p.H * p.W) * p.C + c4 * 4;
        f32x4 u[4][6];
#pragma unroll
        for (int j = 0; j < 6; ++j) {
            f32x4 d[4];
            const int x = x0 + j;
#pragma unroll
            for (int i = 0; i < 4; ++i) {
                const int y = y0 + i;
                const bool ok = (unsigned)y < (unsigned)p.H && (unsigned)x < (unsigned)p.W && (j < 4 || two);
                const f32x4 raw = ok ? *reinterpret_cast<const f32x4*>(img + ((size_t)y * p.W + x) * p.C) : f32x4{0.f, 0.f, 0.f, 0.f};
                d[i] = epi::split_decode4(raw);
            }
            column(u, j, d);
        }
        emit(s, u);
    } else {
        const f32x4 sc4 = *reinterpret_cast<const f32x4*>(p.src.scale + c4 * 4), sf4 = *reinterpret_cast<const f32x4*>(p.src.shift + c4 * 4);
        const float slope = (p.src.flags & EPI_LEAKY) ? 0.1f : 1.f;
        float vmax = 0.f;
        auto finish = [&](const f32x4 a4, const uint32_t gs, const int i, const int j) __attribute__((always_inline)) -> f32x4 {
            bool keep[4] = {true, true, true, true};
            if constexpr (DROP != 0) {
                const uint64_t pix = ((uint64_t)gs * p.H + (uint32_t)(y0 + 1)) * p.W + (uint32_t)(x0 + 1);
                const int64_t off = (int64_t)(((i - 1) * p.W + (j - 1)) * p.C);
                const epi::DropRow drow(p.src.idx_base + pix * (uint64_t)p.C + (uint64_t)(c4 * 4) + (uint64_t)off, p.src.k1);
                if constexpr (DROP == 2) {
                    const uint32_t el = drow.el_lo();
                    const uint32_t w = p.src.mask_bits[el >> 5] >> (el & 31u);
#pragma unroll
                    for (int k = 0; k < 4; ++k) keep[k] = (w >> k) & 1u;
                } else epi::keep4(drow, 0, p.src.k0, p.src.thr, keep);
            }
            const f32x4 v = epi::bn_act4(a4, sc4, sf4, keep, slope);
            vmax = epi::absmax4(vmax, v);
            return epi::split_decode4(epi::split_encode4(v));
        };
        if constexpr (FEED == 1) {
            const uint32_t il = fdiv(s, d_nsl), slice = s - il * nsl, image = img_lo + il, T = (uint32_t)p.src_T;
            uint32_t ga = image * T + slice * (uint32_t)BYOLO_WS_FEED_SLICE, gb = ga + (uint32_t)BYOLO_WS_FEED_SLICE;
            gb = gb < (image + 1u) * T ? gb : (image + 1u) * T;
            ga = ga > (uint32_t)p.s0 ? ga : (uint32_t)p.s0;
            const uint32_t s_end = (uint32_t)p.s0 + (uint32_t)p.P / (uint32_t)(p.th * p.tw);
            gb = gb < s_end ? gb : s_end;
            if (ga >= gb) return;
            const float* img = p.src_low + ((size_t)image * p.H * p.W) * p.C + c4 * 4;
            f32x4 acc[4][4];
#pragma unroll
            for (int j = 0; j < 4; ++j)
#pragma unroll
                for (int i = 0; i < 4; ++i) {
                    const int y = y0 + i, x = x0 + j;
                    const bool ok = (unsigned)y < (unsigned)p.H && (unsigned)x < (unsigned)p.W;
                    acc[i][j] = ok ? *reinterpret_cast<const f32x4*>(img + ((size_t)y * p.W + x) * p.C) : f32x4{0.f, 0.f, 0.f, 0.f};
                }
#pragma unroll 1
            for (uint32_t gs = ga; gs < gb; ++gs) {
                f32x4 u[4][6];
#pragma unroll
                for (int j = 0; j < 4; ++j) {
                    f32x4 d[4];
                    const int x = x0 + j;
#pragma unroll
                    for (int i = 0; i < 4; ++i) {
                        const int y = y0 + i;
                        const bool ok = (unsigned)y < (unsigned)p.H && (unsigned)x < (unsigned)p.W;
                        d[i] = ok ? finish(acc[i][j], gs, i, j) : f32x4{0.f, 0.f, 0.f, 0.f};
                    }
                    column(u, j, d);
                }
                emit_tile(gs - (uint32_t)p.s0, u, 0);
            }
        } else {
            const uint32_t gs = (uint32_t)p.s0 + s, lh = (uint32_t)p.H >> 1, lw = (uint32_t)p.W >> 1;
            const float* low = p.src_low + ((size_t)gs * lh * lw) * p.C + c4 * 4;
            const float* part = p.src_part ? p.src_part + ((size_t)(gs / (uint32_t)p.src_T) * p.H * p.W) * p.C + c4 * 4 : nullptr;
            f32x4 lo[3][4];
#pragma unroll
            for (int a = 0; a < 3; ++a)
#pragma unroll
                for (int b = 0; b < 4; ++b) {
                    const int ly = (int)ty - 1 + a, lx = (int)tx0 - 1 + b;
                    const bool ok = (unsigned)ly < lh && (unsigned)lx < lw && (b < 3 || two);
                    lo[a][b] = ok ? *reinterpret_cast<const f32x4*>(low + ((size_t)ly * lw + lx) * p.C) : f32x4{0.f, 0.f, 0.f, 0.f};
                }
            f32x4 u[4][6];
#pragma unroll
            for (int j = 0; j < 6; ++j) {
                f32x4 d[4];
                const int x = x0 + j;
#pragma unroll
                for (int i = 0; i < 4; ++i) {
                    const int y = y0 + i;
                    const bool ok = (unsigned)y < (unsigned)p.H && (unsigned)x < (unsigned)p.W && (j < 4 || two);
                    f32x4 a4 = lo[(i + 1) >> 1][(j + 1) >> 1];
                    if (ok && part) a4 += *reinterpret_cast<const f32x4*>(part + ((size_t)y * p.W + x) * p.C);
                    d[i] = ok ? finish(a4, gs, i, j) : f32x4{0.f, 0.f, 0.f, 0.f};
                }
                column(u, j, d);
            }
            emit(s, u);
        }
        if (p.src.status && vmax >= 65520.f) { atomicOr(p.src.status, 1u); atomicMin(p.src.status + 1, (unsigned)p.src.layer_idx); }
    }
}

template <int FEED>
static void launch_input_feed(const WinoParams& p, unsigned grid, hipStream_t st, int twp, uint32_t groups, uint32_t img_lo, uint32_t nsl) {
    const FastDiv a = make_fastdiv((uint32_t)twp), b = make_fastdiv((uint32_t)(p.th * twp)), c = make_fastdiv((uint32_t)p.th), d = make_fastdiv(nsl);
    const int drop = !(p.src.flags & EPI_DROPOUT) ? 0 : (p.src.mask_bits ? 2 : 1);
    if constexpr (FEED == 0) hipLaunchKernelGGL((wino_split_input2_kernel<0, 0>), dim3(grid), dim3(256), 0, st, p, a, b, twp, c, groups, img_lo, d, nsl);
    else if (drop == 0) hipLaunchKernelGGL((wino_split_input2_kernel<FEED, 0>), dim3(grid), dim3(256), 0, st, p, a, b, twp, c, groups, img_lo, d, nsl);
    else if (drop == 1) hipLaunchKernelGGL((wino_split_input2_kernel<FEED, 1>), dim3(grid), dim3(256), 0, st, p, a, b, twp, c, groups, img_lo, d, nsl);
    else hipLaunchKernelGGL((wino_split_input2_kernel<FEED, 2>), dim3(grid), dim3(256), 0, st, p, a, b, twp, c, groups, img_lo, d, nsl);
}

hipError_t launch_wino_split_input(const WinoParams& p, hipStream_t st) {
    const int twp = p.feed == 1 ? p.tw : (p.tw + 1) / 2;
    const uint32_t ns = (uint32_t)(p.P / (p.th * p.tw));
    uint32_t groups = ns, img_lo = 0, nsl = 1;
    if (p.feed < 0 || p.feed > 2) return hipErrorInvalidValue;
    if (p.feed) {
        if (!p.src_low || !p.src.scale || !p.src.shift || p.src_T < 1 || ns < 1 || (p.feed == 2 && ((p.H | p.W) & 1))) return hipErrorInvalidValue;
    }
    if (p.feed == 1) {
        img_lo = (uint32_t)p.s0 / (uint32_t)p.src_T;
        nsl = ((uint32_t)p.src_T + BYOLO_WS_FEED_SLICE - 1) / BYOLO_WS_FEED_SLICE;
        groups = (((uint32_t)p.s0 + ns - 1) / (uint32_t)p.src_T - img_lo + 1) * nsl;
    }
    const uint64_t rows = (uint64_t)groups * p.th * twp + (uint64_t)(p.P_pad - p.P);
    const uint64_t total = rows * (uint64_t)(p.C >> 2);
    const unsigned grid = (unsigned)((total + 255) / 256);
    if (p.feed == 0) launch_input_feed<0>(p, grid, st, twp, groups, img_lo, nsl);
    else if (p.feed == 1) launch_input_feed<1>(p, grid, st, twp, groups, img_lo, nsl);
    else launch_input_feed<2>(p, grid, st, twp, groups, img_lo, nsl);
    return hipGetLastError();
}

__host__ __device__ constexpr int wino_cA(int a, int i) { return a == 0 ? (i < 3 ? 1 : 0) : (i == 0 ? 0 : (i == 1 ? 1 : -1)); }

template <int WINO_BN>
__global__ __launch_bounds__(WINO_BN * 2, 2) void wino_split_kernel(const WinoSplitParams p) {
    extern __shared__ __attribute__((aligned(16))) float smem[];
    __shared__ uint32_t s_claim;
    constexpr int WINO_BM = 64;
    using BT = SplitTile<WINO_BM, WINO_BN, 1, WINO_BN / 32>;
    constexpr int TM = BT::TM, A_LD = BT::A_LD;
    static_assert(BT::TN == 1, "one 32-column block per wave");
    const BT bt(smem);

    const uint32_t nwg = gridDim.x, xcd = blockIdx.x & 7u, slot = blockIdx.x >> 3;
    const uint32_t n_units = (uint32_t)p.units, uq = n_units >> 3, ur = n_units & 7u;
    const uint32_t x0 = xcd * uq + (xcd < ur ? xcd : ur), xn = uq + (xcd < ur ? 1u : 0u);
    const uint32_t ustep = (nwg >> 3) + (xcd < (nwg & 7u) ? 1u : 0u);
    if (slot >= xn) return;
    const uint32_t n_tiles = (uint32_t)p.n_tiles;
    auto unit_of = [&](uint32_t k, uint32_t& rt, uint32_t& ct) __attribute__((always_inline)) { const uint32_t u = x0 + k; rt = fdiv(u, p.d_ntiles); ct = u - rt * n_tiles; };
    auto voff_of = [&](uint32_t rt, uint32_t (&v)[A_LD]) __attribute__((always_inline)) {
#pragma unroll
        for (int j = 0; j < A_LD; ++j) {
            const uint32_t row = (uint32_t)bt.a_r + (uint32_t)(BT::NT / 8) * j;
            if constexpr (BYOLO_WS_V_KTMAJOR != 0) v[j] = rt * (uint32_t)WINO_BM * (uint32_t)p.C * 4u + (row * 32u + (uint32_t)bt.a_q * 4u) * 4u;
            else v[j] = ((rt * (uint32_t)WINO_BM + row) * (uint32_t)p.C + (uint32_t)bt.a_q * 4u) * 4u;
        }
    };
    const __amdgpu_buffer_rsrc_t a_rsrc = make_rsrc(p.v, p.v_bytes);
    const __amdgpu_buffer_rsrc_t w_rsrc = make_rsrc(p.w, p.w_bytes);
    const uint32_t KT = (uint32_t)p.KT;
    const uint32_t w_step = (uint32_t)p.N * BK * 4;

    constexpr int NSET = WINO_BN == 256 ? 4 : 2;
    f32x4 a_reg[NSET][A_LD];
    f16x8 bfr[2][2][1][2];
    uint32_t a_voff[A_LD];
    voff_of(0u, a_voff);
    uint32_t a_base, a_soff, a_kt = 0, a_pt = 0, a_xi_base = 0, a_next_base = 0, a_has_next = 0;
    uint32_t w_soff = 0;
    const uint32_t rt_bytes = (uint32_t)WINO_BM * (uint32_t)p.C * 4u;
    { uint32_t rt, ct; unit_of(slot, rt, ct); a_base = rt * rt_bytes; a_soff = a_base; }
    auto load_a = [&](auto set_tag) __attribute__((always_inline)) {
#pragma unroll
        for (int j = 0; j < A_LD; ++j) a_reg[decltype(set_tag)::value][j] = buffer_load_x4(a_rsrc, a_voff[j], a_soff);
        ++a_kt;
        const uint32_t wrap = a_kt == KT ? 1u : 0u;
        a_kt = wrap ? 0u : a_kt;
        a_xi_base += wrap ? p.xi_stride : 0u;
        a_pt += wrap;
        const uint32_t roll = (a_pt == 16u ? 1u : 0u) & a_has_next;
        a_pt = roll ? 0u : a_pt;
        a_xi_base = roll ? 0u : a_xi_base;
        a_base = roll ? a_next_base : a_base;
        a_soff = a_base + a_xi_base + a_kt * (BYOLO_WS_V_KTMAJOR != 0 ? WINO_BM * BK * 4 : BK * 4);
    };
    auto load_b = [&](auto set_tag) __attribute__((always_inline)) { bt.load_b(bfr[decltype(set_tag)::value], w_rsrc, w_soff); w_soff += w_step; };

    f32x16 Y[4][TM], M[TM][1];
    using c0 = std::integral_constant<int, 0>;
    using c1 = std::integral_constant<int, 1>;
    using c2 = std::integral_constant<int, 2>;
    using c3 = std::integral_constant<int, 3>;
    f16x8 af0[TM][2], af1[TM][2];
    load_a(c0{});
    bt.template store_a<0>(a_reg[0]);
    if constexpr (NSET == 4) { load_a(c1{}); load_a(c2{}); load_a(c3{}); load_a(c0{}); }
    else { load_a(c1{}); load_a(c0{}); }
    __syncthreads();

    auto ktile = [&](auto buf_tag, auto set_tag, auto first_tag) __attribute__((always_inline)) {
        constexpr int BUF = decltype(buf_tag)::value;
        using ST = decltype(set_tag);
        pipe::tile_body_split<BUF, true, (WS_ABL & 1) ? 0 : BT::NBF, (WS_ABL & 4) ? 0 : A_LD, (WS_ABL & 4) ? 0 : A_LD, ((WS_ABL & 16) ? 4 : 0) | ((WS_ABL & 32) ? 8 : 0), decltype(first_tag)::value>(
            bt, M, af0, af1, bfr[(WS_ABL & 1) ? 0 : BUF], [&]() __attribute__((always_inline)) { load_b(std::integral_constant<int, BUF ^ 1>{}); },
            [&]() __attribute__((always_inline)) { load_a(ST{}); }, [&]() __attribute__((always_inline)) { if constexpr (!(WS_ABL & 4)) bt.template store_a<BUF ^ 1>(a_reg[ST::value]); });
    };
    auto run_point = [&]() __attribute__((always_inline)) {
        constexpr std::true_type first{};
        constexpr std::false_type later{};
        if constexpr (NSET == 4) {
            ktile(c0{}, c1{}, first); ktile(c1{}, c2{}, later); ktile(c0{}, c3{}, later); ktile(c1{}, c0{}, later);
            for (uint32_t kt = 4; kt < KT; kt += 4) { ktile(c0{}, c1{}, later); ktile(c1{}, c2{}, later); ktile(c0{}, c3{}, later); ktile(c1{}, c0{}, later); }
        } else {
            ktile(c0{}, c1{}, first); ktile(c1{}, c0{}, later);
            for (uint32_t kt = 2; kt < KT; kt += 2) { ktile(c0{}, c1{}, later); ktile(c1{}, c0{}, later); }
        }
    };
    typedef float f32x2 __attribute__((ext_vector_type(2)));

    auto epilogue = [&](auto mode_tag, uint32_t rt, uint32_t ct) __attribute__((always_inline)) {
        constexpr int MODE = decltype(mode_tag)::value;
        const float slope = (p.epi.flags & EPI_LEAKY) ? 0.1f : 1.f;
        const uint32_t tt = (uint32_t)(p.th * p.tw);
        int tid_e = (int)threadIdx.x;
        asm volatile("" : "+v"(tid_e));
        const int e_wn = tid_e >> 6, e_li = tid_e & 31, e_lh = (tid_e >> 5) & 1;
        const int nb = (int)(ct * WINO_BN) + e_wn * 32 + 4 * e_lh;
        float vmax = 0.f;
        f32x4 sc4[4], sf4[4];
#pragma unroll
        for (int g = 0; g < 4; ++g) {
            sc4[g] = *reinterpret_cast<const f32x4*>(p.epi.scale + nb + 8 * g);
            sf4[g] = *reinterpret_cast<const f32x4*>(p.epi.shift + nb + 8 * g);
        }
#pragma unroll
        for (int i = 0; i < TM; ++i) {
            const uint32_t t = rt * (uint32_t)WINO_BM + (uint32_t)i * 32u + (uint32_t)e_li;
            if (t >= (uint32_t)p.P) continue;
            const uint32_t s = fdiv(t, p.d_tt), r = t - s * tt;
            const uint32_t ty = fdiv(r, p.d_tw), tx = r - ty * (uint32_t)p.tw;
#pragma unroll
            for (int o = 0; o < 4; ++o) {
                const uint32_t oy = 2 * ty + (o >> 1), ox = 2 * tx + (o & 1);
                if (oy >= (uint32_t)p.H || ox >= (uint32_t)p.W) continue;
                const uint64_t pix = ((uint64_t)(p.s0 + s) * p.H + oy) * p.W + ox;
                const uint64_t idx_row = p.epi.idx_base + pix * (uint64_t)p.N + (uint64_t)nb;
                const epi::DropRow drow(idx_row, p.epi.k1);
                float* d = p.y + (size_t)pix * p.N + nb;
#pragma unroll
                for (int g = 0; g < 4; ++g) {
                    const int dn = 8 * g;
                    f32x4 a4;
#pragma unroll
                    for (int q = 0; q < 4; ++q) a4[q] = Y[o][i][4 * g + q];
                    bool keep[4] = {true, true, true, true};
                    if constexpr (MODE == 2) {
                        const uint32_t el = drow.el_lo() + (uint32_t)dn;
                        const uint32_t w = p.epi.mask_bits[el >> 5] >> (el & 31u);
#pragma unroll
                        for (int q = 0; q < 4; ++q) keep[q] = (w >> q) & 1u;
                    } else if constexpr (MODE == 1) epi::keep4(drow, dn, p.epi.k0, p.epi.thr, keep);
                    const f32x4 v = epi::bn_act4_pk(a4, sc4[g], sf4[g], keep, slope);
                    vmax = epi::absmax4(vmax, v);
                    *reinterpret_cast<f32x4*>(d + dn) = epi::split_encode4(v);
                }
            }
        }
        if (p.epi.status && vmax >= 65520.f) { atomicOr(p.epi.status, 1u); atomicMin(p.epi.status + 1, (unsigned)p.epi.layer_idx); }
    };

    auto epilogue_res = [&](uint32_t rt, uint32_t ct) __attribute__((always_inline)) {
        const float slope = (p.epi.flags & EPI_LEAKY) ? 0.1f : 1.f;
        const uint32_t tt = (uint32_t)(p.th * p.tw);
        int tid_e = (int)threadIdx.x;
        asm volatile("" : "+v"(tid_e));
        const int e_wn = tid_e >> 6, e_li = tid_e & 31, e_lh = (tid_e >> 5) & 1;
        const int nb = (int)(ct * WINO_BN) + e_wn * 32 + 4 * e_lh;
        float vmax = 0.f;
        f32x4 sc4[4], sf4[4];
#pragma unroll
        for (int g = 0; g < 4; ++g) {
            sc4[g] = *reinterpret_cast<const f32x4*>(p.epi.scale + nb + 8 * g);
            sf4[g] = *reinterpret_cast<const f32x4*>(p.epi.shift + nb + 8 * g);
        }
        const bool keep[4] = {true, true, true, true};
        auto row_of = [&](int k, bool& ok) __attribute__((always_inline)) -> size_t {
            const uint32_t t0 = rt * (uint32_t)WINO_BM + (uint32_t)(k >> 2) * 32u + (uint32_t)e_li;
            const uint32_t t = t0 < (uint32_t)p.P ? t0 : (uint32_t)p.P - 1u;
            const uint32_t s = fdiv(t, p.d_tt), r = t - s * tt;
            const uint32_t ty = fdiv(r, p.d_tw), tx = r - ty * (uint32_t)p.tw;
            const uint32_t oy0 = 2 * ty + (uint32_t)((k >> 1) & 1), ox0 = 2 * tx + (uint32_t)(k & 1);
            ok = t0 < (uint32_t)p.P && oy0 < (uint32_t)p.H && ox0 < (uint32_t)p.W;
            const uint32_t oy = oy0 < (uint32_t)p.H ? oy0 : (uint32_t)p.H - 1u, ox = ox0 < (uint32_t)p.W ? ox0 : (uint32_t)p.W - 1u;
            return (size_t)(((uint64_t)(p.s0 + s) * p.H + oy) * p.W + ox) * p.N + nb;
        };
        constexpr int AHEAD = BYOLO_WS_RES_AHEAD;
        f32x4 rr4[AHEAD][4];
        bool okv[AHEAD + 1]; size_t rowv[AHEAD + 1];
#pragma unroll
        for (int a = 0; a < AHEAD; ++a) {
            rowv[a] = row_of(a, okv[a]);
#pragma unroll
            for (int g = 0; g < 4; ++g) rr4[a][g] = *reinterpret_cast<const f32x4*>(p.residual + rowv[a] + 8 * g);
        }
#pragma unroll
        for (int k = 0; k < 4 * TM; ++k) {
            if (k + AHEAD < 4 * TM) rowv[AHEAD] = row_of(k + AHEAD, okv[AHEAD]);
#pragma unroll
            for (int g = 0; g < 4; ++g) {
                f32x4 a4;
#pragma unroll
                for (int q = 0; q < 4; ++q) a4[q] = Y[k & 3][k >> 2][4 * g + q];
                f32x4 v = epi::bn_act4_pk(a4, sc4[g], sf4[g], keep, slope);
                v += epi::split_decode4(rr4[k % AHEAD][g]);
                if (k + AHEAD < 4 * TM) rr4[k % AHEAD][g] = *reinterpret_cast<const f32x4*>(p.residual + rowv[AHEAD] + 8 * g);
                if (okv[0]) {
                    vmax = epi::absmax4(vmax, v);
                    *reinterpret_cast<f32x4*>(p.y + rowv[0] + 8 * g) = epi::split_encode4(v);
                }
            }
#pragma unroll
            for (int a = 0; a < AHEAD; ++a) { okv[a] = okv[a + 1]; rowv[a] = rowv[a + 1]; }
        }
        if (p.epi.status && vmax >= 65520.f) { atomicOr(p.epi.status, 1u); atomicMin(p.epi.status + 1, (unsigned)p.epi.layer_idx); }
    };

    const bool dyn = p.persist == 2;
    for (uint32_t k = slot, k_next; k < xn; k = k_next) {
        uint32_t rt, ct; unit_of(k, rt, ct);
        k_next = k + ustep;
        if (dyn) { if (threadIdx.x == 0) s_claim = ustep + atomicAdd(p.claims + xcd, 1u); a_has_next = 0; }
        else {
            a_has_next = k_next < xn ? 1u : 0u;
            uint32_t rt2, ct2; unit_of(a_has_next ? k_next : k, rt2, ct2); a_next_base = rt2 * rt_bytes;
        }
        __builtin_amdgcn_sched_barrier(0);
        w_soff = ct * (WINO_BN / 32) * SPLIT_WBLOCK;
        load_b(c0{});
        bt.template read_frags<0, 0>(af0);
#pragma unroll
        for (int o = 0; o < 4; ++o)
#pragma unroll
            for (int i = 0; i < TM; ++i)
#pragma unroll
                for (int r = 0; r < 16; ++r) Y[o][i][r] = 0.f;
            for (int xi = 0; xi < 16; ++xi) {
                run_point();
                if (dyn && xi == 0) {
                    k_next = (uint32_t)__builtin_amdgcn_readfirstlane((int)*reinterpret_cast<volatile uint32_t*>(&s_claim));
                    a_has_next = k_next < xn ? 1u : 0u;
                    uint32_t rt2, ct2; unit_of(a_has_next ? k_next : k, rt2, ct2); a_next_base = rt2 * rt_bytes;
                }
                if constexpr (WS_ABL & 2) { if (xi != 15) continue; }
                const int I = xi >> 2, J = xi & 3;
#pragma unroll
                for (int o = 0; o < 4; ++o) {
                    const float c = (float)(wino_cA(o >> 1, I) * wino_cA(o & 1, J));
                    if constexpr (WS_FOLD_SKIP) { if (c == 0.f) continue; }
                    const f32x2 cc = {c, c};
#pragma unroll
                    for (int i = 0; i < TM; ++i)
#pragma unroll
                        for (int r = 0; r < 16; r += 2) {
                            const f32x2 y2 = __builtin_elementwise_fma(cc, f32x2{M[i][0][r], M[i][0][r + 1]}, f32x2{Y[o][i][r], Y[o][i][r + 1]});
                            Y[o][i][r] = y2[0]; Y[o][i][r + 1] = y2[1];
                        }
                }
            }
        if (p.residual) epilogue_res(rt, ct);
        else if (!(p.epi.flags & EPI_DROPOUT)) epilogue(std::integral_constant<int, 0>{}, rt, ct);
        else if (p.epi.mask_bits) epilogue(std::integral_constant<int, 2>{}, rt, ct);
        else epilogue(std::integral_constant<int, 1>{}, rt, ct);
    }
}

bool wino_split_ok(int C, int N) { return C >= 128 && (C % 128) == 0 && N >= 128 && (N % 128) == 0; }

template <int WINO_BN>
static hipError_t launch_wino_split_bn(const WinoSplitParams& p, hipStream_t st) {
    using BT = SplitTile<64, WINO_BN, 1, WINO_BN / 32>;
    auto k = wino_split_kernel<WINO_BN>;
    static std::atomic<uint64_t> attr_done{0};
    if (hipError_t e = set_dynamic_lds_once(reinterpret_cast<const void*>(k), BT::LDS_BYTES, attr_done); e != hipSuccess) return e;
    const int resident = 256 * (WINO_BN == 256 ? 1 : 2);
    const int grid = (p.persist && p.units > resident) ? resident : p.units;
    hipLaunchKernelGGL(k, dim3((unsigned)grid), dim3(WINO_BN * 2), BT::LDS_BYTES, st, p);
    return hipGetLastError();
}
hipError_t launch_wino_split(const WinoSplitParams& p, hipStream_t st) {
    if (p.bm != 64 || (p.residual && (p.epi.flags & EPI_DROPOUT))) return hipErrorInvalidValue;
    return p.bn == 256 ? launch_wino_split_bn<256>(p, st) : launch_wino_split_bn<128>(p, st);
}

}
```

### include/byolo.h

```cpp
#ifndef BYOLO_H_
#define BYOLO_H_

#include <stddef.h>
#include <stdint.h>

#ifdef __cplusplus
extern "C" {
#endif

#define BYOLO_API __attribute__((visibility("default")))

#define BYOLO_OK 0
#define BYOLO_ERR_ARG (-1)
#define BYOLO_ERR_STATE (-2)
#define BYOLO_ERR_HIP (-3)
#define BYOLO_ERR_NOMEM (-4)
#define BYOLO_ERR_RANGE (-5)

typedef struct byolo byolo_t;

enum { BYOLO_DET_STANDARD = 0, BYOLO_DET_ALEATORIC = 1, BYOLO_DET_EPISTEMIC = 2 };
enum { BYOLO_NMS_AGNOSTIC = 0, BYOLO_NMS_TWO_CLASS = 1, BYOLO_NMS_PER_CLASS = 2 };
#define BYOLO_NMS_MAX_CLASSES 128
enum { BYOLO_NORM_BN = 1, BYOLO_NORM_DROPOUT = 2 };

typedef struct byolo_cfg {
    int32_t img_h, img_w, img_c;
    int32_t cls_cnt;
    float   drop_prob;
    int32_t max_out;
    float   iou_thresh;
    int32_t nms_mode;
    int32_t keep_all_outputs;
} byolo_cfg;

BYOLO_API int32_t byolo_create(const byolo_cfg* cfg, int32_t device, byolo_t** out);
BYOLO_API int32_t byolo_destroy(byolo_t* h);
enum { BYOLO_PREC_F32 = 0, BYOLO_PREC_SPLIT_F16 = 1 };
BYOLO_API int32_t byolo_set_precision(byolo_t* h, int32_t precision);
BYOLO_API int32_t byolo_get_precision(const byolo_t* h);
BYOLO_API const char* byolo_precision_note(const byolo_t* h);
BYOLO_API const char* byolo_last_error(const byolo_t* h);
BYOLO_API const char* byolo_version(void);
#define BYOLO_ABI_VERSION 7
BYOLO_API int32_t byolo_abi_version(void);

typedef struct byolo_plan_opts {
    int32_t struct_bytes;
    int32_t graphs;
    int32_t serialize_convs;
    int32_t serialize_heads;
    int32_t dedup;
    int32_t lowmain;
    int32_t kx3, p1;
    int32_t b2b;
    int32_t kx3_wide;
    int32_t wino_split;
    int32_t wino_split_min_c;
    int32_t wino_split_bn;
    int32_t wino_split_rounds;
    int32_t winograd;
    int32_t wino_fused;
    int32_t stream1x1;
    int32_t gemm_stream;
    int32_t ksplit;
    int32_t streamk;
    int32_t plain_epilogue;
    int32_t wshift_per_layer;
    int32_t nms_general;
    int32_t wino_split_persist;
    int32_t wino_split_feed;
    float   wino_split_min_gflop;
    float   wino_split_chunk_mb;
    float   wino_min_gflop;
    float   wino_chunk_mb;
    float   wino_min_ratio;
} byolo_plan_opts;
BYOLO_API int32_t byolo_get_plan_opts(const byolo_t* h, byolo_plan_opts* out);
BYOLO_API int32_t byolo_set_plan_opts(byolo_t* h, const byolo_plan_opts* opts);
BYOLO_API int32_t byolo_graph_stats(const byolo_t* h, int32_t* n_graphs, int64_t* replays, int64_t* captures, int64_t* updates);


BYOLO_API int32_t byolo_add_conv(byolo_t* h, const char* scope, int32_t filters, int32_t ksize, int32_t stride,
                       int32_t norm_flags);
BYOLO_API int32_t byolo_add_residual(byolo_t* h, int32_t shortcut);
BYOLO_API int32_t byolo_add_route(byolo_t* h, const int32_t* routes, int32_t n_routes);
BYOLO_API int32_t byolo_add_upsample(byolo_t* h);
BYOLO_API int32_t byolo_add_stack(byolo_t* h, int32_t src);
BYOLO_API int32_t byolo_add_detection(byolo_t* h, const char* scope, int32_t kind, const float* priors_hw );

BYOLO_API int32_t byolo_mark_backbone_end(byolo_t* h);

BYOLO_API int32_t byolo_num_params(const byolo_t* h);
BYOLO_API int32_t byolo_param_info(const byolo_t* h, int32_t i, const char** name, int32_t* ndim, int64_t shape[4]);
BYOLO_API int32_t byolo_set_param(byolo_t* h, const char* name, const float* h_data, int64_t count);
BYOLO_API int32_t byolo_get_param(const byolo_t* h, const char* name, float* h_data, int64_t count);
BYOLO_API int32_t byolo_finalize(byolo_t* h);

BYOLO_API int32_t byolo_num_layers(const byolo_t* h);
BYOLO_API int32_t byolo_num_boxes(const byolo_t* h, int64_t* n_boxes, int32_t* row_len);
BYOLO_API int32_t byolo_workspace_bytes(byolo_t* h, int32_t B, int32_t T, size_t* out);
BYOLO_API int32_t byolo_plan_num(byolo_t* h, int32_t B, int32_t T, int32_t inject, int32_t* n_steps, int32_t* n_tensors, int64_t* arena_bytes);
BYOLO_API int32_t byolo_plan_step(byolo_t* h, int32_t step, int32_t* out_tensor, int32_t* fuses_next, int32_t reads[8], int32_t* n_reads);
BYOLO_API int32_t byolo_plan_tensor(byolo_t* h, int32_t tensor, int64_t* offset, int64_t* bytes, int32_t* read_after_the_steps);
BYOLO_API int32_t byolo_forward(byolo_t* h, const float* d_img, int32_t B, int32_t T, uint64_t seed, int32_t dropout_on,
                      const uint32_t* d_mask_bits, void* d_workspace, size_t workspace_bytes,
                      float* d_boxes, float* d_rows, int32_t* d_kept, int32_t* d_count, void* stream);
BYOLO_API int32_t byolo_num_dropout(const byolo_t* h);
BYOLO_API int32_t byolo_mask_layout(byolo_t* h, int32_t B, int32_t T, int32_t ordinal, int64_t* bit_offset, int64_t* elements);
BYOLO_API int32_t byolo_set_async(byolo_t* h, int32_t on);
BYOLO_API int32_t byolo_status(byolo_t* h, void* stream, uint32_t* flags, int32_t* layer);
BYOLO_API int32_t byolo_clear_status(byolo_t* h, void* stream);
BYOLO_API int32_t byolo_set_first_image(byolo_t* h, int64_t first_image);
BYOLO_API int32_t byolo_set_tshard(byolo_t* h, int32_t t0, int32_t T_total);
BYOLO_API int32_t byolo_finish_tshard(byolo_t* h, float* d_sums, int32_t B, int32_t T_total, void* stream);
BYOLO_API int32_t byolo_max_images(byolo_t* h, int32_t T, int32_t* max_images);
BYOLO_API int32_t byolo_layer_output(const byolo_t* h, int32_t idx, const float** d_ptr, int64_t shape[4]);
BYOLO_API int32_t byolo_copy_layer_output(const byolo_t* h, int32_t idx, float* d_dst, int64_t count, void* stream);

BYOLO_API int32_t byolo_decode(byolo_t* h, int32_t kind, const float* d_raw, int32_t B, int32_t T, int32_t lh, int32_t lw,
                     const float* priors_hw , int32_t layer_id, float* d_boxes,
                     int64_t n_total, int64_t box_base, void* stream);
BYOLO_API int32_t byolo_epistemic_stats(byolo_t* h, const float* d_raw, int32_t B, int32_t T, int32_t lh, int32_t lw,
                                        float* d_ev_loc, float* d_epi_covar, float* d_obj_samples, float* d_cls_samples,
                                        void* stream);
BYOLO_API size_t  byolo_nms_workspace_bytes(int32_t B, int64_t N);
BYOLO_API size_t  byolo_nms_workspace_bytes_ex(int32_t B, int64_t N, int32_t nms_mode, int32_t cls_cnt);
BYOLO_API int32_t byolo_nms_class_counts(byolo_t* h, int32_t* d_class_counts, int32_t B, int32_t cls_cnt, void* stream);
BYOLO_API int32_t byolo_sort_nms(byolo_t* h, const float* d_boxes, int32_t B, int64_t N, int32_t D, int32_t obj_idx,
                       int32_t cls_start_idx, int32_t nms_mode, int32_t max_out, float iou_thresh,
                       void* d_sort_ws, size_t ws_bytes,
                       float* d_rows, int32_t* d_kept, int32_t* d_count, void* stream);

BYOLO_API int32_t byolo_encode_gt(byolo_t* h, int32_t n_layers, const int32_t* layer_hw, const double* priors_hw,
                                  const float* d_boxes, const int32_t* d_labels, const int32_t* d_counts, int32_t B,
                                  int32_t max_boxes, float ign_thresh, float* d_loc, float* d_obj, int32_t* d_cls,
                                  float* d_ign, void* d_workspace, size_t workspace_bytes, void* stream);
BYOLO_API size_t  byolo_encode_gt_workspace_bytes(int32_t B, int32_t max_boxes);
BYOLO_API size_t  byolo_loss_workspace_bytes(void);
BYOLO_API int32_t byolo_loss(byolo_t* h, int32_t kind, int32_t aleatoric_loss, int32_t cls_cnt, const float* d_raw, int32_t pitch,
                             int32_t S, int32_t lh, int32_t lw, const float* d_gt_loc, const float* d_gt_obj,
                             const int32_t* d_gt_cls, const float* d_gt_ign, int64_t gt_stride, double* d_loss,
                             float* d_grad, int32_t grad_pitch, void* d_workspace, size_t workspace_bytes, void* stream);

BYOLO_API int32_t byolo_calibrate_bn(byolo_t* h, const float* d_img, int32_t B, void* d_workspace, size_t workspace_bytes,
                           void* stream);

BYOLO_API int32_t byolo_set_profiling(byolo_t* h, int32_t on);
BYOLO_API int32_t byolo_resume_profiling(byolo_t* h, int32_t on);
BYOLO_API int32_t byolo_stage_ms(byolo_t* h, float ms[4]);
BYOLO_API int32_t byolo_set_profile_depth(byolo_t* h, int32_t depth);
BYOLO_API int32_t byolo_select_profile(byolo_t* h, int32_t age);
BYOLO_API int32_t byolo_num_steps(const byolo_t* h);
BYOLO_API int32_t byolo_step_profile(byolo_t* h, int32_t i, int32_t* layer, int32_t* variant, int64_t mnk[3], float* ms,
                                     double* algo_flops);
BYOLO_API int32_t byolo_step_split(byolo_t* h, int32_t i, int32_t* ksplit, int32_t* split_tiles);
BYOLO_API int32_t byolo_flops(byolo_t* h, int32_t B, int32_t T, double* flops);

BYOLO_API uint32_t byolo_crc32c(const void* h_data, size_t n);


BYOLO_API int32_t byolo_normalize_u8(byolo_t* h, const uint8_t* d_u8, int64_t n, float* d_f32, void* stream);

enum { BYOLO_AUG_COLOR_NONE = 0, BYOLO_AUG_SATURATION = 1, BYOLO_AUG_BRIGHTNESS = 2, BYOLO_AUG_HUE = 3 };
enum { BYOLO_AUG_NOISE_NONE = 0, BYOLO_AUG_COLORED_SALT_N_PEPPER = 1, BYOLO_AUG_SALT_N_PEPPER = 2, BYOLO_AUG_GAUSSIAN = 3 };
typedef struct byolo_aug_plan {
    int32_t y0, x0, ch, cw;
    int32_t row0;
    int32_t rescale, flip, blur_k;
    int32_t color_op, noise_op;
    float color_param;
    float noise_param;
    uint64_t noise_key;
} byolo_aug_plan;
BYOLO_API int32_t byolo_augment_batch(byolo_t* h, const uint8_t* d_u8, int32_t B, int32_t src_h, int32_t src_w, int64_t img_stride,
                                      const byolo_aug_plan* h_plans, int32_t out_h, int32_t out_w, float* d_out, void* stream);

BYOLO_API int32_t byolo_copy_status(byolo_t* h, uint32_t* d_out, void* stream);

enum { BYOLO_PNG_OK = 0, BYOLO_PNG_UNSUPPORTED = 1, BYOLO_PNG_SHAPE = 2, BYOLO_PNG_CORRUPT = 3 };
BYOLO_API int32_t byolo_png_decode_batch(const uint8_t* const* h_png, const size_t* png_bytes, int32_t n, int32_t img_h,
                                         int32_t img_w, int32_t img_c, uint8_t* h_out, int32_t threads, int32_t* status,
                                         int32_t* found_shape);

enum { BYOLO_FEED_IO = 4, BYOLO_FEED_CRC = 5, BYOLO_FEED_PROTO = 6 };
BYOLO_API int32_t byolo_feed_records(const int32_t* fds, const int64_t* offsets, const int64_t* lengths, int32_t n, int32_t verify_crc,
                                     int32_t img_h, int32_t img_w, int32_t img_c, uint8_t* h_out, int32_t threads, char* h_names,
                                     int32_t name_cap, int32_t* status, int32_t* found_shape);

BYOLO_API int64_t byolo_format_ecp_json(int32_t kind, const float* h_rows, int32_t n_rows, int32_t row_len, int32_t img_h,
                                        int32_t img_w, int32_t cls_cnt, int32_t obj_idx, int32_t cls_start,
                                        int32_t implicit_background, const char* const* labels, int32_t n_labels,
                                        char* h_out, size_t cap);

typedef struct byolo_trainer byolo_trainer_t;
BYOLO_API int32_t byolo_trainer_create(byolo_t* h, int32_t aleatoric_loss, byolo_trainer_t** out);
BYOLO_API int32_t byolo_trainer_destroy(byolo_trainer_t* tr);
BYOLO_API int32_t byolo_trainer_set_fallback(byolo_trainer_t* tr, byolo_t* h_f32);
BYOLO_API int32_t byolo_trainer_workspace_bytes(byolo_trainer_t* tr, int32_t B, size_t* bytes);
BYOLO_API int32_t byolo_trainer_step(byolo_trainer_t* tr, const float* d_img, int32_t B, uint64_t seed, const uint32_t* d_mask_bits,
                                     const float* d_gt_loc, const float* d_gt_obj, const int32_t* d_gt_cls, const float* d_gt_ign,
                                     float lr, int32_t grads_only, double* d_losses, void* d_workspace, size_t workspace_bytes,
                                     void* stream);
BYOLO_API int32_t byolo_trainer_num_vars(const byolo_trainer_t* tr);
BYOLO_API int32_t byolo_trainer_var_info(const byolo_trainer_t* tr, int32_t i, const char** name, int32_t* ndim, int64_t shape[4]);
BYOLO_API int32_t byolo_trainer_get(byolo_trainer_t* tr, const char* name, int32_t slot, float* h_data, int64_t count);
BYOLO_API int32_t byolo_trainer_set(byolo_trainer_t* tr, const char* name, int32_t slot, const float* h_data, int64_t count);
BYOLO_API int32_t byolo_trainer_get_step(const byolo_trainer_t* tr, int64_t* step);
BYOLO_API int32_t byolo_trainer_set_step(byolo_trainer_t* tr, int64_t step);
BYOLO_API int32_t byolo_trainer_export(byolo_trainer_t* tr, byolo_t* dst);
BYOLO_API int32_t byolo_trainer_taps(const byolo_trainer_t* tr, int32_t* layers, int32_t cap);
BYOLO_API int32_t byolo_trainer_layer_output(byolo_trainer_t* tr, int32_t layer, float* d_dst, int64_t count, int64_t shape[4],
                                             void* stream);

#define BYOLO_EVAL_MAX_GT 1024
#define BYOLO_EVAL_MAX_UNC 16
#define BYOLO_EVAL_RECORD_HEAD 7
typedef struct byolo_eval byolo_eval_t;
typedef struct byolo_eval_cfg {
    int32_t struct_bytes;
    int32_t row_len, obj_idx, cls_start_idx, cls_cnt;
    int32_t n_unc;
    int32_t unc_cols[BYOLO_EVAL_MAX_UNC];
    float iou_thresh, min_score;
// ... 145 lines not shown
```

Measured before the change: 380.3.

## Group Winograd tiles into edge classes to skip unused transform points

For odd-sized feature maps, Winograd F(2x2,3x3) tiles are split into four classes (interior, right edge, bottom edge, corner) and each class gets its own contiguous, padded segment of slots. The split-f16 GEMM kernel then skips the transform points and output accumulations that partial edge tiles never use, and the input transform skips storing those points. The planner's cost model is scaled by the fraction of points kept. In exchange there is more index arithmetic in the epilogue and input kernel, extra padding per class, and a new template variant.

```diff
diff --git a/bayesian-yolov3_amd/byolo/_lib.py b/bayesian-yolov3_amd/byolo/_lib.py
--- a/bayesian-yolov3_amd/byolo/_lib.py
+++ b/bayesian-yolov3_amd/byolo/_lib.py
@@ -29,7 +29,7 @@
     _fields_ = [(n, ctypes.c_int32) for n in (
         "struct_bytes", "graphs", "serialize_convs", "serialize_heads", "dedup", "lowmain", "kx3", "p1", "b2b", "kx3_wide", "wino_split", "wino_split_min_c",
         "wino_split_bn", "wino_split_rounds", "winograd", "wino_fused", "stream1x1", "gemm_stream", "ksplit", "streamk",
-        "plain_epilogue", "wshift_per_layer", "nms_general", "wino_split_persist", "wino_split_feed")] + [(n, ctypes.c_float) for n in (
+        "plain_epilogue", "wshift_per_layer", "nms_general", "wino_split_persist", "wino_split_feed", "wino_split_classes")] + [(n, ctypes.c_float) for n in (
         "wino_split_min_gflop", "wino_split_chunk_mb", "wino_min_gflop", "wino_chunk_mb", "wino_min_ratio")]
 
 
diff --git a/bayesian-yolov3_amd/csrc/byolo_api.hip b/bayesian-yolov3_amd/csrc/byolo_api.hip
--- a/bayesian-yolov3_amd/csrc/byolo_api.hip
+++ b/bayesian-yolov3_amd/csrc/byolo_api.hip
@@ -46,7 +46,7 @@
     o.struct_bytes = (int32_t)sizeof o;
     o.graphs = 1; o.serialize_convs = 1; o.serialize_heads = 1; o.dedup = 1; o.lowmain = 1; o.kx3 = 1; o.p1 = 1; o.b2b = 1; o.kx3_wide = 0;
     o.wino_split = 1; o.wino_split_min_c = 256; o.wino_split_bn = 0; o.wino_split_rounds = 0;
-    o.winograd = 1; o.wino_fused = 1; o.stream1x1 = 1; o.gemm_stream = 1; o.ksplit = -1; o.streamk = 1; o.plain_epilogue = 1; o.wino_split_persist = 0; o.wino_split_feed = 3;
+    o.winograd = 1; o.wino_fused = 1; o.stream1x1 = 1; o.gemm_stream = 1; o.ksplit = -1; o.streamk = 1; o.plain_epilogue = 1; o.wino_split_persist = 0; o.wino_split_feed = 3; o.wino_split_classes = 1;
     o.wino_split_min_gflop = 30.f; o.wino_split_chunk_mb = 1500.f; o.wino_min_gflop = 10.f; o.wino_chunk_mb = 800.f; o.wino_min_ratio = 80.f;
 }
 static void plan_opts_from_env(byolo_plan_opts& o) {
@@ -58,7 +58,7 @@
     geti("BYOLO_WINO_SPLIT", o.wino_split); geti("BYOLO_WINO_SPLIT_MIN_C", o.wino_split_min_c); geti("BYOLO_WINO_SPLIT_BN", o.wino_split_bn);
     geti("BYOLO_WINO_SPLIT_ROUNDS", o.wino_split_rounds); geti("BYOLO_WINOGRAD", o.winograd);
     geti("BYOLO_WINO_FUSED", o.wino_fused); geti("BYOLO_STREAM1X1", o.stream1x1); geti("BYOLO_GEMM_STREAM", o.gemm_stream);
-    geti("BYOLO_KSPLIT", o.ksplit); geti("BYOLO_STREAMK", o.streamk); geti("BYOLO_PLAIN_EPILOGUE", o.plain_epilogue); geti("BYOLO_WINO_SPLIT_PERSIST", o.wino_split_persist); geti("BYOLO_WINO_SPLIT_FEED", o.wino_split_feed);
+    geti("BYOLO_KSPLIT", o.ksplit); geti("BYOLO_STREAMK", o.streamk); geti("BYOLO_PLAIN_EPILOGUE", o.plain_epilogue); geti("BYOLO_WINO_SPLIT_PERSIST", o.wino_split_persist); geti("BYOLO_WINO_SPLIT_FEED", o.wino_split_feed); geti("BYOLO_WINO_SPLIT_CLASSES", o.wino_split_classes);
     geti("BYOLO_WSHIFT_PER_LAYER", o.wshift_per_layer); geti("BYOLO_NMS_GENERAL", o.nms_general);
     getf("BYOLO_WINO_SPLIT_MIN_GFLOP", o.wino_split_min_gflop); getf("BYOLO_WINO_SPLIT_CHUNK_MB", o.wino_split_chunk_mb);
     getf("BYOLO_WINO_MIN_GFLOP", o.wino_min_gflop); getf("BYOLO_WINO_CHUNK_MB", o.wino_chunk_mb); getf("BYOLO_WINO_MIN_RATIO", o.wino_min_ratio);
@@ -85,7 +85,7 @@
     if (o->graphs < 0 || o->graphs > 2 || o->serialize_convs < 0 || o->serialize_convs > 2 || o->b2b < 0 || o->b2b > 2 || o->kx3_wide < 0 || o->kx3_wide > 2 ||
         o->wino_split < 0 || o->wino_split > 2 || o->winograd < 0 || o->winograd > 2 || o->wino_fused < 0 || o->wino_fused > 2 || o->stream1x1 < 0 || o->stream1x1 > 2 ||
         o->streamk < 0 || o->streamk > 2 || o->ksplit < -1 || o->ksplit > 64 || (o->wino_split_bn != 0 && o->wino_split_bn != 128 && o->wino_split_bn != 256) ||
-        o->wino_split_rounds < 0 || o->wino_split_persist < 0 || o->wino_split_persist > 2 || o->wino_split_feed < 0 || o->wino_split_feed > 3 || !(o->wino_split_chunk_mb > 0.f) || !(o->wino_chunk_mb > 0.f) || !(o->wino_split_min_gflop >= 0.f) || !(o->wino_min_gflop >= 0.f) || !(o->wino_min_ratio >= 0.f))
+        o->wino_split_rounds < 0 || o->wino_split_persist < 0 || o->wino_split_persist > 2 || o->wino_split_feed < 0 || o->wino_split_feed > 3 || o->wino_split_classes < 0 || o->wino_split_classes > 1 || !(o->wino_split_chunk_mb > 0.f) || !(o->wino_chunk_mb > 0.f) || !(o->wino_split_min_gflop >= 0.f) || !(o->wino_min_gflop >= 0.f) || !(o->wino_min_ratio >= 0.f))
         return fail(h, BYOLO_ERR_ARG, "byolo_set_plan_opts: a field outside its range (include/byolo.h)");
     const byolo_plan_opts& c = h->opts;
     const bool repack = (o->wshift_per_layer != 0) != (c.wshift_per_layer != 0) || (o->dedup != 0) != (c.dedup != 0) || (o->lowmain != 0) != (c.lowmain != 0) || (o->kx3 != 0) != (c.kx3 != 0) || (o->p1 != 0) != (c.p1 != 0);
@@ -711,7 +711,8 @@
         if (feed) w = *feed;
         w.x = feed ? nullptr : c.src0; w.v = V;
         w.H = l.H; w.W = l.W; w.C = c.C0; w.N = c.N; w.th = wp.th; w.tw = wp.tw;
-        w.s0 = s0; w.P = ns * tt; w.P_pad = (int)align_up((size_t)w.P, 128);
+        w.cls = wino_classes(ns, l.H, l.W, h->opts.wino_split_classes != 0);
+        w.s0 = s0; w.P = ns * tt; w.P_pad = (int)w.cls.slots;
         w.d_tt = make_fastdiv((uint32_t)tt); w.d_tw = make_fastdiv((uint32_t)wp.tw);
         w.d_c4 = make_fastdiv((uint32_t)(c.C0 / 4)); w.d_n4 = make_fastdiv((uint32_t)(c.N / 4));
         w.vmul = 1.f / ACT_SCALE;
@@ -724,7 +725,7 @@
         f.y = c.dst; f.residual = (c.epi.flags & EPI_RESIDUAL) ? c.residual : nullptr;
         f.epi = c.epi; f.epi.scale = dptr(h, drop ? l.wscalek_off : l.wscale_off);
         f.C = c.C0; f.N = c.N; f.KT = c.C0 / 32; f.n_tiles = c.N / wp.bn; f.bn = wp.bn;
-        f.H = l.H; f.W = l.W; f.th = wp.th; f.tw = wp.tw; f.s0 = s0; f.P = w.P; f.P_pad = w.P_pad;
+        f.H = l.H; f.W = l.W; f.th = wp.th; f.tw = wp.tw; f.s0 = s0; f.P = w.P; f.P_pad = w.P_pad; f.cls = w.cls;
         f.bm = wp.bm; f.units = (w.P_pad / wp.bm) * f.n_tiles;
         const int chunk_idx = s0 / wp.chunk;
         f.persist = (h->opts.wino_split_persist == 2 && c.counters && chunk_idx < CNT_PER_STEP / 8) ? 2 : (h->opts.wino_split_persist ? 1 : 0);
diff --git a/bayesian-yolov3_amd/csrc/byolo_kernels.h b/bayesian-yolov3_amd/csrc/byolo_kernels.h
--- a/bayesian-yolov3_amd/csrc/byolo_kernels.h
+++ b/bayesian-yolov3_amd/csrc/byolo_kernels.h
@@ -81,6 +81,38 @@
     int f_N, f_Npad, f_ldc;
 };
 
+#ifndef BYOLO_WS_CLASSES
+#define BYOLO_WS_CLASSES 1
+#endif
+struct WinoClasses {
+    uint32_t start[4];
+    uint32_t fill[4];
+    uint32_t n[4];
+    FastDiv d_n[4], d_twi;
+    uint32_t thi, twi;
+    uint32_t slots;
+    uint32_t on;
+};
+inline WinoClasses wino_classes(int samples, int H, int W, bool enable) {
+    WinoClasses k;
+    const uint32_t th = (uint32_t)(H + 1) / 2, tw = (uint32_t)(W + 1) / 2, S = (uint32_t)samples;
+    const bool on = BYOLO_WS_CLASSES != 0 && enable && ((H | W) & 1);
+    k.thi = on ? (uint32_t)H / 2 : th; k.twi = on ? (uint32_t)W / 2 : tw; k.on = on ? 1u : 0u;
+    uint32_t at = 0;
+    for (uint32_t c = 0; c < 4; ++c) {
+        k.n[c] = ((c & 2u) ? th - k.thi : k.thi) * ((c & 1u) ? tw - k.twi : k.twi);
+        k.d_n[c] = make_fastdiv(k.n[c] ? k.n[c] : 1u);
+        k.start[c] = at; k.fill[c] = at + S * k.n[c];
+        at = (k.fill[c] + 63u) & ~63u;
+    }
+    k.d_twi = make_fastdiv(k.twi ? k.twi : 1u);
+    k.slots = on ? at : (S * th * tw + 127u) & ~127u;
+    if (!on) for (uint32_t c = 1; c < 4; ++c) k.start[c] = k.fill[c] = k.slots;
+    return k;
+}
+__host__ __device__ constexpr uint32_t wino_class_points(uint32_t c) { return ((c & 1u) ? 0x7777u : 0xFFFFu) & ((c & 2u) ? 0x0FFFu : 0xFFFFu); }
+__host__ __device__ constexpr uint32_t wino_class_outputs(uint32_t c) { return ((c & 1u) ? 0x5u : 0xFu) & ((c & 2u) ? 0x3u : 0xFu); }
+
 struct WinoParams {
     const float* x; float* v;
     const float* m; float* y;
@@ -94,6 +126,7 @@
     int feed, src_T;
     const float* src_low; const float* src_part;
     EpiArgs src;
+    WinoClasses cls;
 };
 struct WinoSplitParams {
     const float* v; uint32_t v_bytes;
@@ -109,6 +142,7 @@
     unsigned* claims;
     int units;
     FastDiv d_ntiles, d_tt, d_tw;
+    WinoClasses cls;
 };
 bool wino_split_ok(int C, int N);
 hipError_t launch_wino_split_input(const WinoParams& p, hipStream_t st);
diff --git a/bayesian-yolov3_amd/csrc/byolo_plan.hip b/bayesian-yolov3_amd/csrc/byolo_plan.hip
--- a/bayesian-yolov3_amd/csrc/byolo_plan.hip
+++ b/bayesian-yolov3_amd/csrc/byolo_plan.hip
@@ -107,7 +107,14 @@
             const double per_sample = 16.0 * th * tw * l.Cin * 4.0;
             const int nchunks = std::max(1, (int)std::ceil(S * per_sample / budget));
             const int chunk = (S + nchunks - 1) / nchunks;
-            const int64_t row_tiles = (int64_t)align_up((size_t)chunk * th * tw, 128) / bm;
+            const bool classes = h->opts.wino_split_classes != 0;
+            auto class_share = [&](const WinoClasses& k) -> double {
+                double pts = 0.0;
+                for (uint32_t c = 0; c < 4; ++c) pts += (double)(((c < 3 ? k.start[c + 1] : k.slots) - k.start[c]) / 64u) * __builtin_popcount(wino_class_points(c));
+                return k.on ? pts / (16.0 * (k.slots / 64u)) : 1.0;
+            };
+            const WinoClasses kc = wino_classes(chunk, l.H, l.W, classes);
+            const int64_t row_tiles = (int64_t)kc.slots / bm;
             const bool can256 = (l.filters % 256) == 0;
             int bn = (bn_pref == 256 && can256) ? 256 : bn_pref == 128 ? 128 : 0;
             if (bn_pref == 256 && !can256) bn = 128;
@@ -115,7 +122,7 @@
             if (bn == 0) bn = t256 <= t128 ? 256 : 128;
             if (on < 2) {
                 const double t_res = l.fused_residual >= 0 ? 4.0 * M * l.filters / 2.5e9 : 0.0;
-                const double t_wino = nchunks * ((bn == 256 ? t256 : t128) + 0.012 + (double)row_tiles * bm * per_sample / ((double)th * tw) / 4.5e9) + t_res;
+                const double t_wino = nchunks * ((bn == 256 ? t256 : t128) * class_share(kc) + 0.012 + (double)row_tiles * bm * per_sample / ((double)th * tw) / 4.5e9) + t_res;
                 const double t_direct = 0.028 + flops / ((l.Cin >= 512 ? 390.0 : 425.0) * 1e9);
                 if (t_wino > 0.97 * t_direct) continue;
             }
@@ -129,10 +136,10 @@
                 const int64_t row_tiles = (int64_t)rounds * slots / n_tiles;
                 const int tt = w.th * w.tw;
                 int c = (int)((row_tiles * w.bm) / tt);
-                while (c > 1 && (int64_t)align_up((size_t)c * tt, 128) / w.bm * n_tiles > (int64_t)rounds * slots) --c;
+                while (c > 1 && (int64_t)wino_classes(c, l.H, l.W, classes).slots / w.bm * n_tiles > (int64_t)rounds * slots) --c;
                 w.chunk = std::max(1, std::min(S, c));
             }
-            const size_t P_pad = align_up((size_t)w.chunk * w.th * w.tw, 128);
+            const size_t P_pad = wino_classes(w.chunk, l.H, l.W, classes).slots;
             w.v_bytes = align_up((size_t)16 * P_pad * l.Cin * 4, 256);
             if (w.v_bytes > CONV_MAX_SRC_BYTES) { w = WinoPlan{}; continue; }
             w.m_bytes = 0;
diff --git a/bayesian-yolov3_amd/csrc/wino_split.hip b/bayesian-yolov3_amd/csrc/wino_split.hip
--- a/bayesian-yolov3_amd/csrc/wino_split.hip
+++ b/bayesian-yolov3_amd/csrc/wino_split.hip
@@ -17,6 +17,7 @@
 #define BYOLO_WS_FOLD_SKIP 1
 #endif
 static constexpr bool WS_FOLD_SKIP = BYOLO_WS_FOLD_SKIP != 0;
+static constexpr bool WS_CLASSES = BYOLO_WS_CLASSES != 0;
 #ifndef BYOLO_WS_RES_AHEAD
 #define BYOLO_WS_RES_AHEAD 1
 #endif
@@ -41,7 +42,7 @@
 #ifndef BYOLO_WS_FEED_SLICE
 #define BYOLO_WS_FEED_SLICE 5
 #endif
-template <int FEED, int DROP>
+template <int FEED, int DROP, bool CLS>
 __global__ __launch_bounds__(256) void wino_split_input2_kernel(const WinoParams p, const FastDiv d_twp, const FastDiv d_ttp, const int twp, const FastDiv d_th,
                                                                 const uint32_t groups, const uint32_t img_lo, const FastDiv d_nsl, const uint32_t nsl) {
     const uint32_t gid = blockIdx.x * 256u + threadIdx.x;
@@ -50,8 +51,15 @@
     const size_t xi_stride = (size_t)p.P_pad * p.C;
     const uint32_t ttp = (uint32_t)(p.th * twp), n_pairs = groups * ttp;
     if (q >= n_pairs) {
-        const uint32_t t = (uint32_t)p.P + (q - n_pairs);
-        if (t >= (uint32_t)p.P_pad) return;
+        uint32_t j = q - n_pairs, t = 0;
+        bool found = false;
+#pragma unroll
+        for (int c = 0; c < 4; ++c) {
+            const uint32_t gap = (c < 3 ? p.cls.start[c < 3 ? c + 1 : 3] : p.cls.slots) - p.cls.fill[c];
+            if (!found && j < gap) { t = p.cls.fill[c] + j; found = true; }
+            else if (!found) j -= gap;
+        }
+        if (!found) return;
         float* v = p.v + v_index(t, c4 * 4, (uint32_t)p.C);
 #pragma unroll
         for (int k = 0; k < 16; ++k) vstore(v + (size_t)k * xi_stride, f32x4{0.f, 0.f, 0.f, 0.f});
@@ -67,15 +75,20 @@
     const int y0 = 2 * (int)ty - 1, x0 = 2 * (int)tx0 - 1;
     const float m = p.vmul;
     auto emit_tile = [&](const uint32_t sl, const f32x4 (&u)[4][6], const int k) __attribute__((always_inline)) {
-        const uint32_t t0 = ((sl * (uint32_t)p.th + ty) * (uint32_t)p.tw + tx0);
-        float* v = p.v + v_index(t0 + (uint32_t)k, c4 * 4, (uint32_t)p.C);
+        const uint32_t tx = tx0 + (uint32_t)k;
+        const bool rgt = CLS && tx >= p.cls.twi, bot = CLS && ty >= p.cls.thi;
+        const uint32_t seg = bot ? (rgt ? p.cls.start[3] : p.cls.start[2]) : (rgt ? p.cls.start[1] : p.cls.start[0]);
+        const uint32_t per = bot ? (rgt ? p.cls.n[3] : p.cls.n[2]) : (rgt ? p.cls.n[1] : p.cls.n[0]);
+        const uint32_t t = seg + sl * per + (bot ? 0u : ty) * (rgt ? 1u : p.cls.twi) + (rgt ? 0u : tx);
+        float* v = p.v + v_index(t, c4 * 4, (uint32_t)p.C);
         const int o = 2 * k;
 #pragma unroll
         for (int i = 0; i < 4; ++i) {
+            if (i == 3 && bot) continue;
             vstore(v + (size_t)(i * 4 + 0) * xi_stride, epi::split_encode4((u[i][o + 0] - u[i][o + 2]) * m));
             vstore(v + (size_t)(i * 4 + 1) * xi_stride, epi::split_encode4((u[i][o + 1] + u[i][o + 2]) * m));
             vstore(v + (size_t)(i * 4 + 2) * xi_stride, epi::split_encode4((u[i][o + 2] - u[i][o + 1]) * m));
-            vstore(v + (size_t)(i * 4 + 3) * xi_stride, epi::split_encode4((u[i][o + 1] - u[i][o + 3]) * m));
+            if (!rgt) vstore(v + (size_t)(i * 4 + 3) * xi_stride, epi::split_encode4((u[i][o + 1] - u[i][o + 3]) * m));
         }
     };
     auto emit = [&](const uint32_t sl, const f32x4 (&u)[4][6]) __attribute__((always_inline)) {
@@ -195,14 +208,14 @@
     }
 }
 
-template <int FEED>
+template <int FEED, bool CLS>
 static void launch_input_feed(const WinoParams& p, unsigned grid, hipStream_t st, int twp, uint32_t groups, uint32_t img_lo, uint32_t nsl) {
     const FastDiv a = make_fastdiv((uint32_t)twp), b = make_fastdiv((uint32_t)(p.th * twp)), c = make_fastdiv((uint32_t)p.th), d = make_fastdiv(nsl);
     const int drop = !(p.src.flags & EPI_DROPOUT) ? 0 : (p.src.mask_bits ? 2 : 1);
-    if constexpr (FEED == 0) hipLaunchKernelGGL((wino_split_input2_kernel<0, 0>), dim3(grid), dim3(256), 0, st, p, a, b, twp, c, groups, img_lo, d, nsl);
-    else if (drop == 0) hipLaunchKernelGGL((wino_split_input2_kernel<FEED, 0>), dim3(grid), dim3(256), 0, st, p, a, b, twp, c, groups, img_lo, d, nsl);
-    else if (drop == 1) hipLaunchKernelGGL((wino_split_input2_kernel<FEED, 1>), dim3(grid), dim3(256), 0, st, p, a, b, twp, c, groups, img_lo, d, nsl);
-    else hipLaunchKernelGGL((wino_split_input2_kernel<FEED, 2>), dim3(grid), dim3(256), 0, st, p, a, b, twp, c, groups, img_lo, d, nsl);
+    if constexpr (FEED == 0) hipLaunchKernelGGL((wino_split_input2_kernel<0, 0, CLS>), dim3(grid), dim3(256), 0, st, p, a, b, twp, c, groups, img_lo, d, nsl);
+    else if (drop == 0) hipLaunchKernelGGL((wino_split_input2_kernel<FEED, 0, CLS>), dim3(grid), dim3(256), 0, st, p, a, b, twp, c, groups, img_lo, d, nsl);
+    else if (drop == 1) hipLaunchKernelGGL((wino_split_input2_kernel<FEED, 1, CLS>), dim3(grid), dim3(256), 0, st, p, a, b, twp, c, groups, img_lo, d, nsl);
+    else hipLaunchKernelGGL((wino_split_input2_kernel<FEED, 2, CLS>), dim3(grid), dim3(256), 0, st, p, a, b, twp, c, groups, img_lo, d, nsl);
 }
 
 hipError_t launch_wino_split_input(const WinoParams& p, hipStream_t st) {
@@ -221,15 +234,20 @@
     const uint64_t rows = (uint64_t)groups * p.th * twp + (uint64_t)(p.P_pad - p.P);
     const uint64_t total = rows * (uint64_t)(p.C >> 2);
     const unsigned grid = (unsigned)((total + 255) / 256);
-    if (p.feed == 0) launch_input_feed<0>(p, grid, st, twp, groups, img_lo, nsl);
-    else if (p.feed == 1) launch_input_feed<1>(p, grid, st, twp, groups, img_lo, nsl);
-    else launch_input_feed<2>(p, grid, st, twp, groups, img_lo, nsl);
+    auto go = [&](auto cls_tag) {
+        constexpr bool CLS = decltype(cls_tag)::value;
+        if (p.feed == 0) launch_input_feed<0, CLS>(p, grid, st, twp, groups, img_lo, nsl);
+        else if (p.feed == 1) launch_input_feed<1, CLS>(p, grid, st, twp, groups, img_lo, nsl);
+        else launch_input_feed<2, CLS>(p, grid, st, twp, groups, img_lo, nsl);
+    };
+    if (p.cls.on) { if constexpr (WS_CLASSES) go(std::true_type{}); else return hipErrorInvalidValue; }
+    else go(std::false_type{});
     return hipGetLastError();
 }
 
 __host__ __device__ constexpr int wino_cA(int a, int i) { return a == 0 ? (i < 3 ? 1 : 0) : (i == 0 ? 0 : (i == 1 ? 1 : -1)); }
 
-template <int WINO_BN>
+template <int WINO_BN, bool CLS>
 __global__ __launch_bounds__(WINO_BN * 2, 2) void wino_split_kernel(const WinoSplitParams p) {
     extern __shared__ __attribute__((aligned(16))) float smem[];
     __shared__ uint32_t s_claim;
@@ -245,7 +263,22 @@
     const uint32_t ustep = (nwg >> 3) + (xcd < (nwg & 7u) ? 1u : 0u);
     if (slot >= xn) return;
     const uint32_t n_tiles = (uint32_t)p.n_tiles;
-    auto unit_of = [&](uint32_t k, uint32_t& rt, uint32_t& ct) __attribute__((always_inline)) { const uint32_t u = x0 + k; rt = fdiv(u, p.d_ntiles); ct = u - rt * n_tiles; };
+    constexpr bool deal = CLS;
+    const uint32_t n_rt = (uint32_t)p.P_pad / 64u;
+    auto unit_of = [&](uint32_t k, uint32_t& rt, uint32_t& ct) __attribute__((always_inline)) {
+        if constexpr (deal) {
+            const uint32_t q = fdiv(k, p.d_ntiles), c0 = k - q * n_tiles;
+            if (8u * q + 8u <= n_rt) { rt = 8u * q + xcd; ct = c0; }
+            else { const uint32_t j = 8u * c0 + xcd, r = fdiv(j, p.d_ntiles); rt = 8u * q + r; ct = j - r * n_tiles; }
+        } else { const uint32_t u = x0 + k; rt = fdiv(u, p.d_ntiles); ct = u - rt * n_tiles; }
+    };
+    auto class_of = [&](uint32_t rt) __attribute__((always_inline)) -> uint32_t {
+        if constexpr (!CLS) return 0u;
+        else {
+            const uint32_t b = rt * 64u;
+            return (b >= p.cls.start[1] ? 1u : 0u) + (b >= p.cls.start[2] ? 1u : 0u) + (b >= p.cls.start[3] ? 1u : 0u);
+        }
+    };
     auto voff_of = [&](uint32_t rt, uint32_t (&v)[A_LD]) __attribute__((always_inline)) {
 #pragma unroll
         for (int j = 0; j < A_LD; ++j) {
@@ -264,25 +297,32 @@
     f16x8 bfr[2][2][1][2];
     uint32_t a_voff[A_LD];
     voff_of(0u, a_voff);
-    uint32_t a_base, a_soff, a_kt = 0, a_pt = 0, a_xi_base = 0, a_next_base = 0, a_has_next = 0;
-    uint32_t w_soff = 0;
+    uint32_t a_base, a_soff, a_kt = 0, a_pt = 0, a_next_base = 0, a_has_next = 0, a_mask = 0xFFFFu, a_next_mask = 0xFFFFu;
+    uint32_t w_soff = 0, w_pt_end = 0, w_next = 0;
     const uint32_t rt_bytes = (uint32_t)WINO_BM * (uint32_t)p.C * 4u;
-    { uint32_t rt, ct; unit_of(slot, rt, ct); a_base = rt * rt_bytes; a_soff = a_base; }
+    { uint32_t rt, ct; unit_of(slot, rt, ct); a_base = rt * rt_bytes; a_soff = a_base; a_mask = wino_class_points(class_of(rt)); }
     auto load_a = [&](auto set_tag) __attribute__((always_inline)) {
 #pragma unroll
         for (int j = 0; j < A_LD; ++j) a_reg[decltype(set_tag)::value][j] = buffer_load_x4(a_rsrc, a_voff[j], a_soff);
         ++a_kt;
         const uint32_t wrap = a_kt == KT ? 1u : 0u;
         a_kt = wrap ? 0u : a_kt;
-        a_xi_base += wrap ? p.xi_stride : 0u;
-        a_pt += wrap;
+        if constexpr (CLS) {
+            const uint32_t rest = a_pt < 16u ? a_mask >> (a_pt + 1u) : 0u;
+            const uint32_t nxt = rest ? a_pt + 1u + (uint32_t)__builtin_ctz(rest) : 16u;
+            a_pt = wrap ? nxt : a_pt;
+        } else a_pt += wrap;
         const uint32_t roll = (a_pt == 16u ? 1u : 0u) & a_has_next;
         a_pt = roll ? 0u : a_pt;
-        a_xi_base = roll ? 0u : a_xi_base;
+        a_mask = roll ? a_next_mask : a_mask;
         a_base = roll ? a_next_base : a_base;
-        a_soff = a_base + a_xi_base + a_kt * (BYOLO_WS_V_KTMAJOR != 0 ? WINO_BM * BK * 4 : BK * 4);
-    };
-    auto load_b = [&](auto set_tag) __attribute__((always_inline)) { bt.load_b(bfr[decltype(set_tag)::value], w_rsrc, w_soff); w_soff += w_step; };
+        a_soff = a_base + a_pt * p.xi_stride + a_kt * (BYOLO_WS_V_KTMAJOR != 0 ? WINO_BM * BK * 4 : BK * 4);
+    };
+    auto load_b = [&](auto set_tag) __attribute__((always_inline)) {
+        bt.load_b(bfr[decltype(set_tag)::value], w_rsrc, w_soff);
+        w_soff += w_step;
+        if constexpr (CLS) w_soff = w_soff == w_pt_end ? w_next : w_soff;
+    };
 
     f32x16 Y[4][TM], M[TM][1];
     using c0 = std::integral_constant<int, 0>;
@@ -316,10 +356,29 @@
     };
     typedef float f32x2 __attribute__((ext_vector_type(2)));
 
+    struct SlotMap { uint32_t start, fill, n, ty0, tx0; FastDiv d_n; bool rgt; };
+    auto slot_map = [&](uint32_t rt) __attribute__((always_inline)) -> SlotMap {
+        const uint32_t c = class_of(rt);
+        const bool rgt = c & 1u, bot = c & 2u;
+        SlotMap m;
+        m.start = bot ? (rgt ? p.cls.start[3] : p.cls.start[2]) : (rgt ? p.cls.start[1] : p.cls.start[0]);
+        m.fill = bot ? (rgt ? p.cls.fill[3] : p.cls.fill[2]) : (rgt ? p.cls.fill[1] : p.cls.fill[0]);
+        m.n = bot ? (rgt ? p.cls.n[3] : p.cls.n[2]) : (rgt ? p.cls.n[1] : p.cls.n[0]);
+        m.d_n = bot ? (rgt ? p.cls.d_n[3] : p.cls.d_n[2]) : (rgt ? p.cls.d_n[1] : p.cls.d_n[0]);
+        m.ty0 = bot ? p.cls.thi : 0u; m.tx0 = rgt ? p.cls.twi : 0u; m.rgt = rgt;
+        return m;
+    };
+    auto tile_of = [&](const SlotMap& m, uint32_t t, uint32_t& s, uint32_t& ty, uint32_t& tx) __attribute__((always_inline)) {
+        const uint32_t l = t - m.start;
+        s = fdiv(l, m.d_n);
+        const uint32_t r = l - s * m.n, q = m.rgt ? r : fdiv(r, p.cls.d_twi);
+        ty = m.ty0 + q; tx = m.tx0 + (m.rgt ? 0u : r - q * p.cls.twi);
+    };
+
     auto epilogue = [&](auto mode_tag, uint32_t rt, uint32_t ct) __attribute__((always_inline)) {
         constexpr int MODE = decltype(mode_tag)::value;
         const float slope = (p.epi.flags & EPI_LEAKY) ? 0.1f : 1.f;
-        const uint32_t tt = (uint32_t)(p.th * p.tw);
+        const SlotMap sm = slot_map(rt);
         int tid_e = (int)threadIdx.x;
         asm volatile("" : "+v"(tid_e));
         const int e_wn = tid_e >> 6, e_li = tid_e & 31, e_lh = (tid_e >> 5) & 1;
@@ -334,9 +393,8 @@
 #pragma unroll
         for (int i = 0; i < TM; ++i) {
             const uint32_t t = rt * (uint32_t)WINO_BM + (uint32_t)i * 32u + (uint32_t)e_li;
-            if (t >= (uint32_t)p.P) continue;
-            const uint32_t s = fdiv(t, p.d_tt), r = t - s * tt;
-            const uint32_t ty = fdiv(r, p.d_tw), tx = r - ty * (uint32_t)p.tw;
+            if (t >= sm.fill) continue;
+            uint32_t s, ty, tx; tile_of(sm, t, s, ty, tx);
 #pragma unroll
             for (int o = 0; o < 4; ++o) {
                 const uint32_t oy = 2 * ty + (o >> 1), ox = 2 * tx + (o & 1);
@@ -369,7 +427,7 @@
 
     auto epilogue_res = [&](uint32_t rt, uint32_t ct) __attribute__((always_inline)) {
         const float slope = (p.epi.flags & EPI_LEAKY) ? 0.1f : 1.f;
-        const uint32_t tt = (uint32_t)(p.th * p.tw);
+        const SlotMap sm = slot_map(rt);
         int tid_e = (int)threadIdx.x;
         asm volatile("" : "+v"(tid_e));
         const int e_wn = tid_e >> 6, e_li = tid_e & 31, e_lh = (tid_e >> 5) & 1;
@@ -384,11 +442,10 @@
         const bool keep[4] = {true, true, true, true};
         auto row_of = [&](int k, bool& ok) __attribute__((always_inline)) -> size_t {
             const uint32_t t0 = rt * (uint32_t)WINO_BM + (uint32_t)(k >> 2) * 32u + (uint32_t)e_li;
-            const uint32_t t = t0 < (uint32_t)p.P ? t0 : (uint32_t)p.P - 1u;
-            const uint32_t s = fdiv(t, p.d_tt), r = t - s * tt;
-            const uint32_t ty = fdiv(r, p.d_tw), tx = r - ty * (uint32_t)p.tw;
+            const uint32_t t = t0 < sm.fill ? t0 : sm.fill - 1u;
+            uint32_t s, ty, tx; tile_of(sm, t, s, ty, tx);
             const uint32_t oy0 = 2 * ty + (uint32_t)((k >> 1) & 1), ox0 = 2 * tx + (uint32_t)(k & 1);
-            ok = t0 < (uint32_t)p.P && oy0 < (uint32_t)p.H && ox0 < (uint32_t)p.W;
+            ok = t0 < sm.fill && oy0 < (uint32_t)p.H && ox0 < (uint32_t)p.W;
             const uint32_t oy = oy0 < (uint32_t)p.H ? oy0 : (uint32_t)p.H - 1u, ox = ox0 < (uint32_t)p.W ? ox0 : (uint32_t)p.W - 1u;
             return (size_t)(((uint64_t)(p.s0 + s) * p.H + oy) * p.W + ox) * p.N + nb;
         };
@@ -430,11 +487,13 @@
         if (dyn) { if (threadIdx.x == 0) s_claim = ustep + atomicAdd(p.claims + xcd, 1u); a_has_next = 0; }
         else {
             a_has_next = k_next < xn ? 1u : 0u;
-            uint32_t rt2, ct2; unit_of(a_has_next ? k_next : k, rt2, ct2); a_next_base = rt2 * rt_bytes;
-        }
+            uint32_t rt2, ct2; unit_of(a_has_next ? k_next : k, rt2, ct2); a_next_base = rt2 * rt_bytes; a_next_mask = wino_class_points(class_of(rt2));
+        }
+        const uint32_t cls = class_of(rt), pmask = wino_class_points(cls), omask = wino_class_outputs(cls);
         __builtin_amdgcn_sched_barrier(0);
-        w_soff = ct * (WINO_BN / 32) * SPLIT_WBLOCK;
-        load_b(c0{});
+        const uint32_t w_unit = ct * (WINO_BN / 32) * SPLIT_WBLOCK;
+        bt.load_b(bfr[0], w_rsrc, w_unit);
+        w_soff = w_unit + w_step;
         bt.template read_frags<0, 0>(af0);
 #pragma unroll
         for (int o = 0; o < 4; ++o)
@@ -443,11 +502,17 @@
 #pragma unroll
                 for (int r = 0; r < 16; ++r) Y[o][i][r] = 0.f;
             for (int xi = 0; xi < 16; ++xi) {
+                if constexpr (CLS) {
+                    if (!((pmask >> xi) & 1u)) continue;
+                    const uint32_t rest = pmask >> (xi + 1), nxt = rest ? (uint32_t)xi + 1u + (uint32_t)__builtin_ctz(rest) : (uint32_t)xi + 1u;
+                    w_pt_end = w_unit + ((uint32_t)xi + 1u) * KT * w_step;
+                    w_next = w_unit + nxt * KT * w_step;
+                }
                 run_point();
                 if (dyn && xi == 0) {
                     k_next = (uint32_t)__builtin_amdgcn_readfirstlane((int)*reinterpret_cast<volatile uint32_t*>(&s_claim));
                     a_has_next = k_next < xn ? 1u : 0u;
-                    uint32_t rt2, ct2; unit_of(a_has_next ? k_next : k, rt2, ct2); a_next_base = rt2 * rt_bytes;
+                    uint32_t rt2, ct2; unit_of(a_has_next ? k_next : k, rt2, ct2); a_next_base = rt2 * rt_bytes; a_next_mask = wino_class_points(class_of(rt2));
                 }
                 if constexpr (WS_ABL & 2) { if (xi != 15) continue; }
                 const int I = xi >> 2, J = xi & 3;
@@ -455,6 +520,7 @@
                 for (int o = 0; o < 4; ++o) {
                     const float c = (float)(wino_cA(o >> 1, I) * wino_cA(o & 1, J));
                     if constexpr (WS_FOLD_SKIP) { if (c == 0.f) continue; }
+                    if constexpr (CLS) { if (!((omask >> o) & 1u)) continue; }
                     const f32x2 cc = {c, c};
 #pragma unroll
                     for (int i = 0; i < TM; ++i)
@@ -474,10 +540,10 @@
 
 bool wino_split_ok(int C, int N) { return C >= 128 && (C % 128) == 0 && N >= 128 && (N % 128) == 0; }
 
-template <int WINO_BN>
+template <int WINO_BN, bool CLS>
 static hipError_t launch_wino_split_bn(const WinoSplitParams& p, hipStream_t st) {
     using BT = SplitTile<64, WINO_BN, 1, WINO_BN / 32>;
-    auto k = wino_split_kernel<WINO_BN>;
+    auto k = wino_split_kernel<WINO_BN, CLS>;
     static std::atomic<uint64_t> attr_done{0};
     if (hipError_t e = set_dynamic_lds_once(reinterpret_cast<const void*>(k), BT::LDS_BYTES, attr_done); e != hipSuccess) return e;
     const int resident = 256 * (WINO_BN == 256 ? 1 : 2);
@@ -487,7 +553,9 @@
 }
 hipError_t launch_wino_split(const WinoSplitParams& p, hipStream_t st) {
     if (p.bm != 64 || (p.residual && (p.epi.flags & EPI_DROPOUT))) return hipErrorInvalidValue;
-    return p.bn == 256 ? launch_wino_split_bn<256>(p, st) : launch_wino_split_bn<128>(p, st);
-}
-
-}
+    if constexpr (WS_CLASSES) { if (p.cls.on) return p.bn == 256 ? launch_wino_split_bn<256, true>(p, st) : launch_wino_split_bn<128, true>(p, st); }
+    else if (p.cls.on) return hipErrorInvalidValue;
+    return p.bn == 256 ? launch_wino_split_bn<256, false>(p, st) : launch_wino_split_bn<128, false>(p, st);
+}
+
+}
diff --git a/include/byolo.h b/include/byolo.h
--- a/include/byolo.h
+++ b/include/byolo.h
@@ -70,6 +70,7 @@
     int32_t nms_general;
     int32_t wino_split_persist;
     int32_t wino_split_feed;
+    int32_t wino_split_classes;
     float   wino_split_min_gflop;
     float   wino_split_chunk_mb;
     float   wino_min_gflop;
```

Result: no change. 383.0 (median of 6 runs) (+0.7%).
